# NVlabs/intrinsic3d

Hardware: AMD Instinct MI355X
Metric: Gauss-Newton iterations/s at the finest SDF level (higher is better)
Workload: dtype f32

## Files before the change

### include/intrinsic3d_hip.h

```cpp
#ifndef INTRINSIC3D_HIP_H
#define INTRINSIC3D_HIP_H
#include <stdint.h>
#ifdef __cplusplus
extern "C" {
#endif

typedef struct i3d_context i3d_context;

typedef enum {
    I3D_OK = 0,
    I3D_ERR_INVALID_ARGUMENT = 1,
    I3D_ERR_NO_DEVICE = 2,
    I3D_ERR_HIP = 3,
    I3D_ERR_STATE = 4,
    I3D_ERR_CAPACITY = 5,
    I3D_ERR_COMM = 6,
    I3D_ERR_IO = 7
} i3d_status;

int  i3d_create(int32_t device_ordinal, i3d_context** out);
void i3d_destroy(i3d_context* ctx);
const char* i3d_last_error(const i3d_context* ctx);
const char* i3d_version(void);

// ... 332 lines not shown

typedef struct {
    i3d_track_sdf_stats base;
    int64_t photo_samples;
    double  photo_rms_initial, photo_rms_final;
} i3d_track_sdf_rgbd_stats;

void i3d_track_sdf_rgbd_desc_default(i3d_track_sdf_rgbd_desc* d);
int  i3d_track_frame_sdf_rgbd(i3d_context* ctx, const i3d_track_sdf_rgbd_desc* desc, int32_t width, int32_t height, const float* depth, const float* luminance,
                              double* pose6_io, i3d_track_sdf_rgbd_stats* stats);
int  i3d_fusion_track_sdf_rgbd(i3d_fusion* f, const i3d_track_sdf_rgbd_desc* desc, int32_t width, int32_t height, const float* depth, const float* luminance,
                               double* pose6_io, i3d_track_sdf_rgbd_stats* stats);
int  i3d_track_frames_sdf_rgbd(i3d_context* ctx, const i3d_track_sdf_rgbd_desc* desc, int32_t num_frames, int32_t width, int32_t height,
                               const float* depth, const float* luminance, double* poses6_io, i3d_track_sdf_rgbd_stats* stats);
int  i3d_track_keyframes_sdf_rgbd(i3d_context* ctx, const i3d_track_sdf_rgbd_desc* desc, int32_t level, int32_t num, const int32_t* frames,
                                  double* poses6_io, i3d_track_sdf_rgbd_stats* stats);

int i3d_comm_unique_id(void* out128, int32_t* bytes);
int i3d_comm_init(i3d_context* ctx, int32_t rank, int32_t world, const void* unique_id, int32_t id_bytes);
void* i3d_comm_sim_create(int32_t world);
void  i3d_comm_sim_destroy(void* shared);
int   i3d_comm_init_sim(i3d_context* ctx, void* shared, int32_t rank);
int   i3d_shard_plan(int32_t A, int32_t world, int32_t rank, const int32_t* anbr, const uint8_t* active,
                     int32_t* chunk, int32_t* own0, int32_t* own1, uint8_t* in_compute_list );
int32_t i3d_shard_vec_index(int32_t a, int32_t chunk, int32_t albedo);
int   i3d_shard_need(int32_t A, int32_t world, const int32_t* anbr , const uint8_t* active , uint64_t* need );
int   i3d_comm_stats(i3d_context* ctx, int64_t* halo_calls, int64_t* halo_bytes_sent, int64_t* reduce_calls, int64_t* reduce_bytes,
                     int32_t* halo_entries_send, int32_t* halo_entries_recv, int32_t* ghost_tiles, int32_t* compute_list);
const char* i3d_comm_transport(i3d_context* ctx);

enum { I3D_K_CLASSIFY = 0, I3D_K_OBSERVE, I3D_K_BUILD, I3D_K_EG_PASS , I3D_K_GATHER, I3D_K_COST, I3D_K_VECTOR, I3D_K_SH,
       I3D_K_EG_AUX ,
       I3D_K_COMM ,
       I3D_K_EG_MR2, I3D_K_EG_MR3 , I3D_K_COUNT };
int i3d_timing_enable(i3d_context* ctx, int32_t on);
int i3d_timing_select(i3d_context* ctx, uint32_t category_mask);
int i3d_timing_get(i3d_context* ctx, double* ms , int64_t* launches , int32_t reset);
int i3d_timing_get_work(i3d_context* ctx, double* ms , int64_t* launches );
int i3d_timing_get_work_ex(i3d_context* ctx, double* ms, int64_t* launches, double* slow_ms , int64_t* slow_launches );
const char* i3d_kernel_name(int32_t k);
int i3d_problem_sizes(i3d_context* ctx, int64_t out[6]);

int i3d_debug_assemble(i3d_context* ctx, const i3d_optimizer_config* cfg, int32_t iteration, int32_t* slots_out);
int64_t i3d_debug_map_order(const int32_t* keys, int64_t n, int32_t mode, int32_t* order);
int i3d_debug_flags(i3d_context* ctx, uint8_t* flags );
int i3d_debug_eg_rows(i3d_context* ctx, int32_t* frame , float* weight ,
                      float* residual , float* jac );
int i3d_debug_reg_rows(i3d_context* ctx, uint8_t* has_er , uint8_t* has_es , float* ea_weight );
int i3d_debug_neighbors(i3d_context* ctx, int32_t* nbr );
int i3d_debug_normal_eq(i3d_context* ctx, double* gradient, double* jtj_diag, double* cost);
int i3d_debug_jtj_apply(i3d_context* ctx, const double* x, double* y);
int i3d_debug_work_list(i3d_context* ctx, int32_t* visit_index , int64_t capacity, int64_t* count);
int i3d_debug_counters(i3d_context* ctx, int64_t* stream_syncs);
int i3d_debug_ladder_stats(i3d_context* ctx, int64_t* out6);
int i3d_debug_ladder_passes(i3d_context* ctx, int64_t* out8);
#define I3D_LM_SCRIPT_GUARD 64
typedef struct i3d_lm_script_desc {
    double cost, ngrad, nfree, radius0;
    int32_t lm_steps;
    int32_t K, fix_poses, fix_intr, fix_dist;
    int32_t n_attempts;
    int32_t n_plan, max_setups;
    const double* cdiag;
    const double* tri;
    const float* tail_c; const float* tail_S;
    const double* xbr; const double* d2xx; const int32_t* pcg_it; const int32_t* pcg_done;
    const double* norms2;
    const double* cand_cost; const int32_t* debug_invalid;
    const int32_t* plan;
} i3d_lm_script_desc;
typedef struct i3d_lm_record { int32_t seq, final_, accepted, pcg_it, termination, kind; double cost, cand_cost, model_change, rel, radius_after, ngrad, nfree; } i3d_lm_record;
int i3d_debug_lm_script(i3d_context* ctx, const i3d_lm_script_desc* script, i3d_lm_record* records , int32_t* n_records, double* state25, int32_t* n_setups,
                        int32_t* setup_meta, double* setup_radius, float* setup_inv_radius, float* setup_blocks, float* setup_d2, float* setup_minv);
int i3d_debug_cull_stats(i3d_context* ctx, int64_t* pairs, int64_t* culled);

int i3d_debug_register_sums(i3d_context* ctx, const i3d_register_desc* desc, int64_t n, const double* points, const double* pose6, const double* pivot3,
                            double* sums29, int64_t* valid);
int i3d_debug_register_row_cap(i3d_context* ctx, int32_t rows);
int i3d_debug_track_sdf_sums(i3d_context* ctx, const i3d_track_sdf_desc* desc, int32_t width, int32_t height, const float* depth,
                             const double* pose6 , const double* pivot3, double* sums29, int64_t* valid, int64_t* valid_pixels);
int i3d_debug_track_batch_frames(i3d_context* ctx, int32_t frames_per_chunk);
int i3d_debug_track_sdf_rgbd_sums(i3d_context* ctx, const i3d_track_sdf_rgbd_desc* desc, int32_t width, int32_t height, const float* depth, const float* luminance,
                                  const double* pose6 , const double* pivot3, double* sums31, int64_t* valid, int64_t* photo_samples);
int i3d_debug_voxel_intensity(i3d_context* ctx, int32_t use_refined_sdf, double* c);
int i3d_fusion_debug_voxel_luminance(i3d_fusion* f, int64_t n, const int32_t* keys , double* c );
int i3d_fusion_debug_track_sdf_rgbd_sums(i3d_fusion* f, const i3d_track_sdf_rgbd_desc* desc, int32_t width, int32_t height, const float* depth,
                                         const float* luminance, const double* pose6 , const double* pivot3, double* sums31, int64_t* valid,
                                         int64_t* photo_samples);
int i3d_fusion_debug_voxels(i3d_fusion* f, int64_t n, const int32_t* keys , uint8_t* found, float* sdf, float* weight, uint8_t* color ,
                            int64_t* first_frame);
int i3d_fusion_debug_frame_samples(i3d_fusion* f, int32_t depth_w, int32_t depth_h, const float* depth_intr4, int32_t color_w, int32_t color_h, const float* color_intr4,
                                   const float* depth, const uint8_t* bgr, const float* pose_cam_to_world16, int32_t erode_window, int64_t n,
                                   const int32_t* keys , uint8_t* on, float* sample, float* wu, uint8_t* has_color, uint8_t* rgb );
int i3d_fusion_debug_register_volume_selection(i3d_fusion* src, const i3d_register_volume_desc* desc, int64_t capacity, int32_t* keys ,
                                               float* sdf , int64_t* count);
int i3d_fusion_debug_register_volume_sums(i3d_fusion* f, i3d_fusion* src, const i3d_register_volume_desc* desc, const double* pose6, const double* pivot3,
                                          int64_t limit, int32_t row_cap, double* sums29, int64_t* valid, int64_t* selected);

#ifdef __cplusplus
}
#endif
#endif
```

### intrinsic3d_amd/binding.py

```python
from __future__ import annotations

import ctypes as C
import os

import numpy as np

_HERE = os.path.dirname(os.path.abspath(__file__))
LIB_PATH = os.environ.get("I3D_LIB") or os.path.join(_HERE, "libintrinsic3d_hip.so")

K_NAMES = ["classify", "observe", "build", "eg_pass", "gather", "cost", "vector", "sh", "eg_aux", "comm", "eg_mr2", "eg_mr3"]


class OptimizerConfig(C.Structure):
    _fields_ = [("iterations", C.c_int32), ("lm_steps", C.c_int32),
                ("lambda_g", C.c_double), ("lambda_r0", C.c_double), ("lambda_r1", C.c_double),
                ("lambda_s0", C.c_double), ("lambda_s1", C.c_double), ("lambda_a", C.c_double),
                ("fix_poses", C.c_int32), ("fix_intrinsics", C.c_int32), ("fix_distortion", C.c_int32),
                ("occlusion_distance", C.c_float), ("num_observations", C.c_int32),
                ("thres_shell", C.c_double), ("grid_level", C.c_int32), ("rgbd_level", C.c_int32),
                ("pcg_fixed_iterations", C.c_int32), ("verbose", C.c_int32), ("carry_trust_radius", C.c_int32), ("fix_sdf", C.c_int32)]


class IterationStats(C.Structure):
    _fields_ = [("rows", C.c_int64 * 4), ("weight_sum", C.c_double * 4), ("type_weight", C.c_double * 4),
# ... 878 lines not shown
        self._check(self.L.i3d_timing_get_work_ex(self.h, _p(ms), _p(n), _p(sms), _p(sn)), "i3d_timing_get_work_ex")
        return {k: (ms[i], int(n[i]), sms[i], int(sn[i])) for i, k in enumerate(K_NAMES)}

    def timing_get(self, reset=True):
        ms = np.zeros(len(K_NAMES)); n = np.zeros(len(K_NAMES), np.int64)
        self._check(self.L.i3d_timing_get(self.h, _p(ms), _p(n), 1 if reset else 0), "i3d_timing_get")
        return {k: (ms[i], int(n[i])) for i, k in enumerate(K_NAMES)}

    def problem_sizes(self):
        o = np.zeros(6, np.int64)
        self._check(self.L.i3d_problem_sizes(self.h, _p(o)), "i3d_problem_sizes")
        return dict(zip(["active", "eg", "er", "es", "ea", "free"], [int(x) for x in o]))

    def debug_assemble(self, cfg, iteration=0):
        s = C.c_int32(0)
        self._check(self.L.i3d_debug_assemble(self.h, C.byref(cfg), int(iteration), C.byref(s)), "i3d_debug_assemble")
        self.slots = s.value
        return s.value

    def debug_flags(self):
        f = np.zeros(self.N, np.uint8)
        self._check(self.L.i3d_debug_flags(self.h, _p(f)), "i3d_debug_flags")
        return f

    def debug_eg_rows(self, jac=True):
        S = self.slots
        fr = np.zeros((self.N, S), np.int32); w = np.zeros((self.N, S), np.float32); r = np.zeros((self.N, S), np.float32)
        J = np.zeros((self.N, S, 29), np.float32) if jac else None
        self._check(self.L.i3d_debug_eg_rows(self.h, _p(fr), _p(w), _p(r), _p(J)), "i3d_debug_eg_rows")
        return fr, w, r, J

    def debug_reg_rows(self):
        er = np.zeros(self.N, np.uint8); es = np.zeros(self.N, np.uint8); ea = np.zeros((self.N, 6), np.float32)
        self._check(self.L.i3d_debug_reg_rows(self.h, _p(er), _p(es), _p(ea)), "i3d_debug_reg_rows")
        return er, es, ea

    def debug_neighbors(self):
        nb = np.zeros((self.N, 18), np.int32)
        self._check(self.L.i3d_debug_neighbors(self.h, _p(nb)), "i3d_debug_neighbors")
        return nb

    def debug_normal_eq(self):
        NP = 2 * self.N + 6 * self.K + 9
        g = np.zeros(NP); d = np.zeros(NP); cost = C.c_double(0)
        self._check(self.L.i3d_debug_normal_eq(self.h, _p(g), _p(d), C.byref(cost)), "i3d_debug_normal_eq")
        return g, d, cost.value

    def debug_counters(self):
        n = C.c_int64(0)
        self._check(self.L.i3d_debug_counters(self.h, C.byref(n)), "i3d_debug_counters")
        return {"stream_syncs": int(n.value)}

    def debug_ladder_stats(self):
        a = (C.c_int64 * 6)()
        self._check(self.L.i3d_debug_ladder_stats(self.h, a), "i3d_debug_ladder_stats")
        return {"batches": int(a[0]), "row_streams": int(a[1]), "system_passes": int(a[2]), "resyncs": int(a[3]), "unused_systems": int(a[4]), "depth": int(a[5])}

    def debug_ladder_passes(self):
        a = (C.c_int64 * 8)()
        self._check(self.L.i3d_debug_ladder_passes(self.h, a), "i3d_debug_ladder_passes")
        return {"live": [int(a[n]) for n in range(7)], "paired": int(a[7])}

    def debug_cull_stats(self):
        a = C.c_int64(0); b = C.c_int64(0)
        self._check(self.L.i3d_debug_cull_stats(self.h, C.byref(a), C.byref(b)), "i3d_debug_cull_stats")
        return int(a.value), int(b.value)

    def debug_jtj_apply(self, x):
        x = np.ascontiguousarray(x, np.float64); y = np.zeros_like(x)
        self._check(self.L.i3d_debug_jtj_apply(self.h, _p(x), _p(y)), "i3d_debug_jtj_apply")
        return y

    def debug_lm_script(self, cost, ngrad, nfree, radius0, lm_steps, attempts, plan=(), K=0, fix=(0, 0, 0), cdiag=None, tri=None, tail_c=None, tail_S=None):
        NS, NB, NT, G = 6 * K + 9, 36 * K + 41, 21 * K + 25, LM_SCRIPT_GUARD
        f64 = lambda a, n, fill: np.full(n, fill, np.float64) if a is None else np.ascontiguousarray(a, np.float64).reshape(n)
        f32 = lambda a, n, fill: np.full(n, fill, np.float32) if a is None else np.ascontiguousarray(a, np.float32).reshape(n)
        cdiag = f64(cdiag, NS, 1.0); tail_c = f32(tail_c, NS, 1.0); tail_S = f32(tail_S, NS, 0.5)
        if tri is None:
            tri = np.zeros(NT); o = 0
            for n in [6] * K + [4, 5]:
                d = 0
                for i in range(n):
                    tri[o + d] = 1.0; d += n - i
                o += n * (n + 1) // 2
        tri = f64(tri, NT, 0.0)
        n = len(attempts["xbr"])
        a = {k: np.ascontiguousarray(attempts[k], np.float64) for k in ("xbr", "d2xx", "norms2", "cand_cost")}
        a.update({k: np.ascontiguousarray(attempts[k], np.int32) for k in ("pcg_it", "pcg_done", "debug_invalid")})
        assert all(a[k].size == (2 * n if k == "norms2" else n) for k in a)
        plan = np.ascontiguousarray(plan, np.int32)
        S = 6 * int(lm_steps) + 6 if plan.size else int(lm_steps)
        d = LmScriptDesc(float(cost), float(ngrad), float(nfree), float(radius0), int(lm_steps), int(K), int(fix[0]), int(fix[1]), int(fix[2]), n, int(plan.size), S,
                         cdiag.ctypes.data, tri.ctypes.data, tail_c.ctypes.data, tail_S.ctypes.data, a["xbr"].ctypes.data, a["d2xx"].ctypes.data, a["pcg_it"].ctypes.data,
                         a["pcg_done"].ctypes.data, a["norms2"].ctypes.data, a["cand_cost"].ctypes.data, a["debug_invalid"].ctypes.data, plan.ctypes.data if plan.size else None)
        rec = np.zeros(128, LM_RECORD_DTYPE); nrec = C.c_int32(0); nset = C.c_int32(0); state = np.zeros(25)
        meta = np.zeros((S, 4), np.int32); radius = np.zeros(S); inv_radius = np.zeros(S, np.float32)
        blocks = np.zeros((S, NB + 2 * G), np.float32); d2 = np.zeros((S, NS + 2 * G), np.float32); minv = np.zeros((S, NS + 2 * G), np.float32)
        self._check(self.L.i3d_debug_lm_script(self.h, C.byref(d), _p(rec), C.addressof(nrec), _p(state), C.addressof(nset), _p(meta), _p(radius), _p(inv_radius),
                                               _p(blocks), _p(d2), _p(minv)), "i3d_debug_lm_script")
        ns = int(nset.value)
        names = ["cost", "radius", "decrease_factor", "ngrad", "nfree", "inv_radius", "done", "termination", "accepted", "invalid", "attempts", "successful", "lad_n"]
        st = {k: state[i] for i, k in enumerate(names)}; st["lad_radius"] = state[13:19].copy(); st["lad_inv_radius"] = state[19:25].copy()
        return {"records": rec[:int(nrec.value)].copy(), "state": st, "meta": meta[:ns], "radius": radius[:ns], "inv_radius": inv_radius[:ns],
                "blocks": blocks[:ns], "d2": d2[:ns], "minv": minv[:ns]}

    def debug_work_list(self):
        n = C.c_int64(0)
        self._check(self.L.i3d_debug_work_list(self.h, None, 0, C.byref(n)), "i3d_debug_work_list")
        out = np.zeros(max(int(n.value), 1), np.int32)
# ... 446 lines not shown
```

### intrinsic3d_amd/csrc/device/build.hip

```cpp
#include <type_traits>
#include "kernels.hpp"
#include "reduce_device.hpp"

namespace i3d {

typedef float v4f_row __attribute__((ext_vector_type(4)));
typedef float v2f_row __attribute__((ext_vector_type(2)));
typedef float f2 __attribute__((ext_vector_type(2)));
static __device__ inline void st_row2(float2* p, float a, float b) { v2f_row v; v.x = a; v.y = b; __builtin_nontemporal_store(v, reinterpret_cast<v2f_row*>(p)); }
static __device__ inline void st_row(float4* p, float a, float b, float c, float d) { v4f_row v; v.x = a; v.y = b; v.z = c; v.w = d; __builtin_nontemporal_store(v, reinterpret_cast<v4f_row*>(p)); }

typedef float f4u __attribute__((ext_vector_type(4), aligned(4)));
typedef const __attribute__((address_space(1))) f4u* gf4u_ptr;
typedef const __attribute__((address_space(1))) float* gf_ptr;

constexpr int Q_LDS_STRIDE = 296;
struct PointShared {
    double P[3];
    double B;
    float n[3];
    float inv_len;
    float s;
    float Ls;
    float dLs[3];
// ... 91 lines not shown
    fold_weights<double>(k.map, wc);
    double fr[4];
#pragma unroll
    for (int i = 0; i < 4; ++i) fr[i] = wc[0] * (double)t[i].x + wc[1] * (double)t[i].y + wc[2] * (double)t[i].z + wc[3] * (double)t[i].w;
    f = wr[0] * fr[0] + wr[1] * fr[1] + wr[2] * fr[2] + wr[3] * fr[3];
    if (WITH_J) {
        float dwc[4], dwr[4]; cr_dweights<float>((float)k.xc, dwc); cr_dweights<float>((float)k.xr, dwr);
        fold_weights<float>(k.map, dwc);
        dfdr = dwr[0] * (float)(fr[0] - fr[1]) + dwr[2] * (float)(fr[2] - fr[1]) + dwr[3] * (float)(fr[3] - fr[1]);
        float acc = 0.0f;
#pragma unroll
        for (int i = 0; i < 4; ++i) acc += (float)wr[i] * (dwc[0] * (t[i].x - t[i].y) + dwc[2] * (t[i].z - t[i].y) + dwc[3] * (t[i].w - t[i].y));
        dfdc = acc;
    }
}

struct PointVal {
    float x0, y0, iz, dfdr, dfdc;
};

template <bool WITH_J>
static __device__ inline bool project_point(const double P[3], const double R[9], const double t[3], const OptParams& p, double& u, double& v, PointVal& o) {
    const double X = R[0] * P[0] + R[1] * P[1] + R[2] * P[2] + t[0];
    const double Y = R[3] * P[0] + R[4] * P[1] + R[5] * P[2] + t[1];
    const double Z = R[6] * P[0] + R[7] * P[1] + R[8] * P[2] + t[2];
    const double ps = p.pyr_scale;
    const double iz = rcp64(Z);
    const double x0 = X * iz, y0 = Y * iz;
    const double r2 = x0 * x0 + y0 * y0, r4 = r2 * r2, r6 = r4 * r2;
    const double dc = 1.0 + p.dist[0] * r2 + p.dist[1] * r4 + p.dist[2] * r6;
    const double xd = x0 * dc + 2.0 * p.dist[3] * x0 * y0 + p.dist[4] * (r2 + 2.0 * x0 * x0);
    const double yd = y0 * dc + 2.0 * p.dist[4] * xd * y0 + p.dist[3] * (r2 + 2.0 * y0 * y0);
    u = (p.intr[0] * ps) * xd + p.intr[2] * ps; v = (p.intr[1] * ps) * yd + p.intr[3] * ps;
    if (WITH_J) { o.x0 = (float)x0; o.y0 = (float)y0; o.iz = (float)iz; }
    return u >= 0.0 && u <= (double)(p.w - 1) && v >= 0.0 && v <= (double)(p.h - 1);
}

static __device__ inline double sdf_to_weight(double sdf, double trunc) {
    const double a = fmin(fabs(sdf), trunc) / trunc;
    return fmin(fmax(1.0 - a, 0.01), 1.0);
}
static __device__ inline float chroma_weight(uchar4 c, uchar4 cn) {
    const float s = 1.0f / 255.0f;
    const float lum = 0.299f * (float)c.x + 0.587f * (float)c.y + 0.114f * (float)c.z;
    const float lumn = 0.299f * (float)cn.x + 0.587f * (float)cn.y + 0.114f * (float)cn.z;
    const float a0 = ((float)c.x * s) / lum - ((float)cn.x * s) / lumn;
    const float a1 = ((float)c.y * s) / lum - ((float)cn.y * s) / lumn;
    const float a2 = ((float)c.z * s) / lum - ((float)cn.z * s) / lumn;
    const float d = sqrtf(a0 * a0 + (a1 * a1 + a2 * a2))      ;
    const float one_minus = 1.0f - d;
    return (one_minus < 0.01f) ? 0.01f : one_minus;
}

template <bool WITH_J, bool FR_LDS, int BATCH> __global__ void k_build(GridView g, RowView r, OptParams p, const FrameConst* __restrict__ frames, double* cost_out, const double* __restrict__ cam9, const LmState* __restrict__ lm);
#ifdef I3D_BUILD_VALUE_PROBE
constexpr int BUILD_PROBE_WAVES = I3D_BUILD_VALUE_PROBE;
#else
constexpr int BUILD_PROBE_WAVES = 0;
#endif
template <bool WITH_J, bool FR_LDS, int BATCH>
__global__ void __launch_bounds__(256, WITH_J ? (BUILD_PROBE_WAVES ? BUILD_PROBE_WAVES : 2) : 3) k_build(GridView g, RowView r, OptParams p, const FrameConst* __restrict__ frames, double* cost_out,
                                                               const double* __restrict__ cam9, const LmState* __restrict__ lm) {
    extern __shared__ double frame_lds_raw[];
    if (!WITH_J) {
        if (lm && lm->done) return;
        if (cam9) { for (int i = 0; i < 4; ++i) p.intr[i] = cam9[i]; for (int i = 0; i < 5; ++i) p.dist[i] = cam9[4 + i]; }
    }
    FrameHot* const flds = reinterpret_cast<FrameHot*>(frame_lds_raw);
    if (FR_LDS) {
        constexpr int WORDS = sizeof(FrameHot) / 8;
        for (int i = threadIdx.x; i < p.K * WORDS; i += blockDim.x) {
            const int f = i / WORDS, w = i - f * WORDS;
            frame_lds_raw[(size_t)f * WORDS + w] = reinterpret_cast<const double*>(&frames[f].hot)[w];
        }
        __syncthreads();
    }
#ifdef I3D_COST_MULTI_PROBE
    int bx = blockIdx.x; bool probe_extra = false;
#ifdef I3D_COST_MULTI_PROBE_FAR
    if (!WITH_J) { constexpr int PB = I3D_COST_MULTI_PROBE; const int per = (int)gridDim.x / PB; probe_extra = (int)blockIdx.x / per != 0; bx = (int)blockIdx.x % per; }
#else
    if (!WITH_J) { constexpr int PB = I3D_COST_MULTI_PROBE; const int grp = (int)blockIdx.x / (8 * PB), rr = (int)blockIdx.x % (8 * PB); probe_extra = rr / 8 != 0; bx = grp * 8 + (rr % 8); }
#endif
    const int ci = bx * blockDim.x + threadIdx.x;
#else
    const int ci = blockIdx.x * blockDim.x + threadIdx.x;
#endif
    const int a = ci < r.nC ? (r.clist ? r.clist[ci] : ci) : -1;
    const bool owned = a >= r.own0 && a < r.own1;
    double cost = 0.0;
    if (a >= 0 && (WITH_J || owned)) {
        const int N = g.N; const size_t Acap = r.Acap;
        const int s = r.alist[a];
        const uint8_t fl = r.aflags[a];
        uint8_t pre_rf = 0, pre_eafree = 0, pre_nrows = 0; float eaw[6] = {0.0f, 0.0f, 0.0f, 0.0f, 0.0f, 0.0f};
        if (!WITH_J) {
            pre_rf = r.regflags[a]; pre_eafree = r.ea_free[a]; pre_nrows = r.nrows[a];
#pragma unroll
            for (int d = 0; d < 6; ++d) eaw[d] = r.ea_w[(size_t)d * Acap + a];
        }
        __builtin_amdgcn_sched_barrier(0);
        if (!(fl & F_ACTIVE)) {
            if (WITH_J) {
                r.regflags[a] = 0; r.ea_free[a] = 0; r.nrows[a] = 0;
                for (int d = 0; d < 6; ++d) r.ea_w[(size_t)d * Acap + a] = 0.0f;
            }
        } else {
        int idx[P_VOX];
        bool eligible = true;
#pragma unroll
        for (int c = 0; c < 10; ++c) { const int nb = slot_fwd_nbr(c); idx[c] = nb < 0 ? s : g.nbr[(size_t)nb * N + s]; eligible &= idx[c] >= 0; }
        idx[10] = idx[0]; idx[11] = idx[6]; idx[12] = idx[1]; idx[13] = idx[4];

        int ring[6];
#pragma unroll
        for (int d = 0; d < 6; ++d) ring[d] = g.nbr[(size_t)d * N + s];
        const bool ring_ok = (fl & F_RING) != 0;
        const double xs = g.x_sdf[s];
        uint8_t rf = 0;
        if (WITH_J) {
            uint8_t nfl[6]; int nrk[6]; uchar4 ncol[6];
#pragma unroll
            for (int d = 0; d < 6; ++d) { const int nb = ring_ok ? ring[d] : s; nfl[d] = g.flags[nb]; nrk[d] = g.rank[nb]; ncol[d] = g.color[nb]; }
            const uchar4 col = g.color[s];
            const int myrank = g.rank[s];
            const double sdf0s = g.sdf0[s];
            if (p.use_er && ring_ok) {
                rf |= 1;
                bool fr = (fl & F_FREE_SDF) != 0;
#pragma unroll
                for (int d = 0; d < 6; ++d) fr |= (nfl[d] & F_FREE_SDF) != 0;
                if (fr) rf |= 8;
            }
            if (p.use_es) { rf |= 2; if ((xs - sdf0s) != 0.0) rf |= 4; if (fl & F_FREE_SDF) rf |= 16; }
            uint8_t eafree = 0;
#pragma unroll
            for (int d = 0; d < 6; ++d) {
                float w = 0.0f;
                if (p.use_ea && ring_ok) {
                    const bool added_before = (nfl[d] & F_ACTIVE) && nrk[d] < myrank;
// ... 191 lines not shown
                    const f2 dyd_dy0 = dc + 2.0f * y0 * y0 * dcr + 2.0f * k4 * (xd + y0 * dxd_dy0) + 6.0f * k3 * y0;
                    const f2 au = dfdc * fxs, av = dfdr * fys;
                    const f2 lx = au * dxd_dx0 + av * dyd_dx0, ly = au * dxd_dy0 + av * dyd_dy0;
                    const f2 L0 = lx * iz, L1 = ly * iz, L2 = -(lx * x0 + ly * y0) * iz;
                    const f2 M0 = L0 * R0 + L1 * R3 + L2 * R6, M1 = L0 * R1 + L1 * R4 + L2 * R7, M2 = L0 * R2 + L1 * R5 + L2 * R8;
                    const f2 c = {cj[ja], cj[jb]};
                    const f2 alb = {q[ja].alb, q[jb].alb}, sv = {q[ja].s, q[jb].s}, il = {q[ja].inv_len, q[jb].inv_len};
                    const f2 n0 = {q[ja].n[0], q[jb].n[0]}, n1 = {q[ja].n[1], q[jb].n[1]}, n2 = {q[ja].n[2], q[jb].n[2]};
                    const f2 v0 = alb * f2{q[ja].dLs[0], q[jb].dLs[0]} + sv * M0, v1 = alb * f2{q[ja].dLs[1], q[jb].dLs[1]} + sv * M1, v2 = alb * f2{q[ja].dLs[2], q[jb].dLs[2]} + sv * M2;
                    const f2 d = n0 * v0 + n1 * v1 + n2 * v2;
                    f2 G0 = (v0 - n0 * d) * il, G1 = (v1 - n1 * d) * il, G2 = (v2 - n2 * d) * il;
                    if (il.x == 0.0f) { G0.x = v0.x; G1.x = v1.x; G2.x = v2.x; }
                    if (il.y == 0.0f) { G0.y = v0.y; G1.y = v1.y; G2.y = v2.y; }
                    const f2 direct = M0 * n0 + M1 * n1 + M2 * n2;
                    const f2 cG0 = c * G0, cG1 = c * G1, cG2 = c * G2, cD = c * (direct - (G0 + G1 + G2)), cLs = c * f2{q[ja].Ls, q[jb].Ls};
                    J[PS[ja][1]] += cG0.x; J[PS[ja][2]] += cG1.x; J[PS[ja][3]] += cG2.x; J[PS[ja][0]] += cD.x; J[P_ALB + ja] = cLs.x;
                    J[PS[jb][1]] += cG0.y; J[PS[jb][2]] += cG1.y; J[PS[jb][3]] += cG2.y; J[PS[jb][0]] += cD.y; J[P_ALB + jb] = cLs.y;
                    const f2 cL0 = c * L0, cL1 = c * L1, cL2 = c * L2;
                    J[P_POSE + 3] -= cL0.x + cL0.y; J[P_POSE + 4] -= cL1.x + cL1.y; J[P_POSE + 5] -= cL2.x + cL2.y;
                    const f2 Px = {(float)q[ja].P[0], (float)q[jb].P[0]}, Py = {(float)q[ja].P[1], (float)q[jb].P[1]}, Pz = {(float)q[ja].P[2], (float)q[jb].P[2]};
                    const f2 wx = c * (Py * M2 - Pz * M1), wy = c * (Pz * M0 - Px * M2), wz = c * (Px * M1 - Py * M0);
                    Wx += wx.x + wx.y; Wy += wy.x + wy.y; Wz += wz.x + wz.y;
                    const f2 cdc = c * dfdc * psf, cdr = c * dfdr * psf;
                    const f2 i0 = cdc * xd, i1 = cdr * yd;
                    J[P_INTR + 0] -= i0.x + i0.y; J[P_INTR + 1] -= i1.x + i1.y; J[P_INTR + 2] -= cdc.x + cdc.y; J[P_INTR + 3] -= cdr.x + cdr.y;
                    const f2 dxk0 = x0 * r2, dxk1 = x0 * r4, dxk2 = x0 * r6, dxk3 = 2.0f * x0 * y0, dxk4 = r2 + 2.0f * x0 * x0;
                    const f2 c2 = 2.0f * k4 * y0;
                    const f2 e0 = c * (au * dxk0 + av * (y0 * r2 + c2 * dxk0)), e1 = c * (au * dxk1 + av * (y0 * r4 + c2 * dxk1)), e2 = c * (au * dxk2 + av * (y0 * r6 + c2 * dxk2));
                    const f2 e3 = c * (au * dxk3 + av * (c2 * dxk3 + (r2 + 2.0f * y0 * y0))), e4 = c * (au * dxk4 + av * (2.0f * xd * y0 + c2 * dxk4));
                    J[P_DIST + 0] -= e0.x + e0.y; J[P_DIST + 1] -= e1.x + e1.y; J[P_DIST + 2] -= e2.x + e2.y; J[P_DIST + 3] -= e3.x + e3.y; J[P_DIST + 4] -= e4.x + e4.y;
                }
                J[P_POSE + 0] = -(Wx * jr[0] + Wy * jr[3] + Wz * jr[6]);
                J[P_POSE + 1] = -(Wx * jr[1] + Wy * jr[4] + Wz * jr[7]);
                J[P_POSE + 2] = -(Wx * jr[2] + Wy * jr[5] + Wz * jr[8]);
                float finz = 0.0f;
#pragma unroll
                for (int i = 0; i < P_TOTAL; ++i) finz = __builtin_fmaf(J[i], 0.0f, finz);
                if (!(finz == 0.0f)) continue;
#pragma unroll
                for (int gq = 0; gq < 7; ++gq)
                    st_row(&r.rows[row_index(a, nout, gq, r.slots)], J[4 * gq], J[4 * gq + 1], J[4 * gq + 2], J[4 * gq + 3]);
                const size_t ro = row_scalar_index(a, nout, r.slots);
                st_row2(&r.row_jt()[row_jt_index(a, nout, r.slots)], J[28], __int_as_float(f | (vox_free ? ROW_FREE_BIT : 0)));
                st_row2(&r.row_wr[ro], roww, (float)res);
                ++nout;
            }
            }
        }
        if (WITH_J) {
            r.nrows[a] = (uint8_t)nout;
        }
        }
    }
#ifdef I3D_COST_MULTI_PROBE
    if (!WITH_J && probe_extra) cost = 0.0;
#endif
    if (!WITH_J) block_partial_d(cost, cost_out, 1, 0);
}

void launch_build(hipStream_t st, GridView g, RowView r, OptParams p, const FrameConst* frames, bool with_jacobian, double* cost_out, double* scratch,
                  const double* cam9, const LmState* lm) {
    if (r.nC <= 0) { if (!with_jacobian && cost_out) (void)hipMemsetAsync(cost_out, 0, sizeof(double), st); return; }
#ifdef I3D_COST_MULTI_PROBE
    const int blocks = with_jacobian ? (r.nC + 255) / 256 : (((r.nC + 255) / 256 + 7) / 8) * 8 * I3D_COST_MULTI_PROBE;
#else
    const int blocks = (r.nC + 255) / 256;
#endif
    double* const cost_dst = cost_out; cost_out = scratch;
    const size_t lds = (size_t)p.K * sizeof(FrameHot), qlds = (size_t)256 * Q_LDS_STRIDE;
    if (with_jacobian) {
#ifdef I3D_BUILD_VALUE_PROBE
        if (BUILD_PROBE_WAVES > 2) {
            if (!set_dynamic_lds((const void*)k_build<true, true, 2>, "k_build<true> value probe", lds, p.K)) return;
            k_build<true, true, 2><<<blocks, 256, lds, st>>>(g, r, p, frames, cost_out, nullptr, nullptr);
            return;
        }
#endif
        if (!set_dynamic_lds((const void*)k_build<true, false, 2>, "k_build<true>", qlds, p.K)) return;
        k_build<true, false, 2><<<blocks, 256, qlds, st>>>(g, r, p, frames, cost_out, nullptr, nullptr);
    } else {
        if (lds <= 48 * 1024) k_build<false, true, 2><<<blocks, 256, lds, st>>>(g, r, p, frames, cost_out, cam9, lm);
        else k_build<false, false, 2><<<blocks, 256, 0, st>>>(g, r, p, frames, cost_out, cam9, lm);
    }
    if (!with_jacobian) launch_reduce_partials(st, scratch, blocks, 1, cost_dst, nullptr, true);
}

template <bool COST>
__global__ void __launch_bounds__(256) k_weight_sums(RowView r, GridView g, double* partials) {
    double s0 = 0, s1 = 0, s2 = 0, s3 = 0, n0 = 0, n3 = 0, na = 0, c0 = 0, c1 = 0, c2 = 0, c3 = 0;
    const int N = g.N;
    for (int a = r.own0 + blockIdx.x * blockDim.x + threadIdx.x; a < r.own1 && a < r.A; a += gridDim.x * blockDim.x) {
        if (!(r.aflags[a] & F_ACTIVE)) continue;
        na += 1.0;
        const int nr = r.nrows[a];
        for (int k = 0; k < nr; ++k) {
            const float2 wr = r.row_wr[row_scalar_index(a, k, r.slots)]; const float w = wr.x;
            s0 += (double)w; if (w != 0.0f) n0 += 1.0;
            if (COST && (__float_as_int(r.row_jt()[row_jt_index(a, k, r.slots)].y) & ROW_FREE_BIT)) c0 += (double)w * ((double)wr.y * (double)wr.y);
        }
        const uint8_t rf = r.regflags[a];
        if (rf & 1) s1 += 1.0;
        if (rf & 2) s2 += 1.0;
        const int s = COST ? r.alist[a] : 0;
        const uint8_t eafree = COST ? r.ea_free[a] : 0;
        const bool er = COST && (rf & 1) && (rf & 8), es = COST && (rf & 2) && (rf & 16);
        int ring[6];
        if (er || eafree) {
#pragma unroll
            for (int d = 0; d < 6; ++d) ring[d] = g.nbr[(size_t)d * N + s];
        }
        if (er || es) {
            const double xs = g.x_sdf[s];
            if (er) {
                const double dxx = g.x_sdf[ring[0]] + g.x_sdf[ring[1]] - 2.0 * xs, dyy = g.x_sdf[ring[2]] + g.x_sdf[ring[3]] - 2.0 * xs, dzz = g.x_sdf[ring[4]] + g.x_sdf[ring[5]] - 2.0 * xs;
                const double lap = dxx + dyy + dzz; c1 += lap * lap;
            }
            if (es) { double e = xs - g.sdf0[s]; if (e == 0.0) e = 0.0000001; c2 += e * e; }
        }
        const double xa = eafree ? g.x_alb[s] : 0.0;
#pragma unroll
        for (int d = 0; d < 6; ++d) {
            const float w = r.ea_w[(size_t)d * r.Acap + a]; s3 += (double)w; if (w != 0.0f) n3 += 1.0;
            if (eafree & (1 << d)) { const double e = xa - g.x_alb[ring[d]]; c3 += (double)w * (e * e); }
        }
    }
    block_partial_d(s0, partials, 13, 0); block_partial_d(s1, partials, 13, 1); block_partial_d(s2, partials, 13, 2); block_partial_d(s3, partials, 13, 3);
    block_partial_d(n0, partials, 13, 4); block_partial_d(0.0, partials, 13, 5); block_partial_d(0.0, partials, 13, 6); block_partial_d(n3, partials, 13, 7);
    block_partial_d(na, partials, 13, 8);
    block_partial_d(c0, partials, 13, 9); block_partial_d(c1, partials, 13, 10); block_partial_d(c2, partials, 13, 11); block_partial_d(c3, partials, 13, 12);
}
void launch_weight_sums(hipStream_t st, RowView r, GridView g, bool with_cost, double* sums13, double* scratch) {
    const int n = r.own1 - r.own0;
    if (n <= 0) return;
    int blocks = (n + 255) / 256; if (blocks > 1024) blocks = 1024;
    if (with_cost) k_weight_sums<true><<<blocks, 256, 0, st>>>(r, g, scratch);
    else k_weight_sums<false><<<blocks, 256, 0, st>>>(r, g, scratch);
    launch_reduce_partials(st, scratch, blocks, 13, sums13, nullptr);
// ... 4 lines not shown
```

### intrinsic3d_amd/csrc/device/common.hpp

```cpp
#pragma once
#include <hip/hip_runtime.h>
#include <cstdint>
#include <cstdio>

namespace i3d {

constexpr int NUM_NBR = 18;
enum Nbr { NB_PX = 0, NB_MX, NB_PY, NB_MY, NB_PZ, NB_MZ, NB_P2X, NB_P2Y, NB_P2Z, NB_PXY, NB_PXZ, NB_PYZ,
           NB_M2X, NB_M2Y, NB_M2Z, NB_MXY, NB_MXZ, NB_MYZ };
__host__ __device__ inline void nbr_offset(int i, int& dx, int& dy, int& dz) {
    constexpr int8_t O[NUM_NBR][3] = {{1,0,0},{-1,0,0},{0,1,0},{0,-1,0},{0,0,1},{0,0,-1},{2,0,0},{0,2,0},{0,0,2},{1,1,0},{1,0,1},{0,1,1},
                                      {-2,0,0},{0,-2,0},{0,0,-2},{-1,-1,0},{-1,0,-1},{0,-1,-1}};
    dx = O[i][0]; dy = O[i][1]; dz = O[i][2];
}

constexpr int P_SDF = 0, P_ALB = 10, P_POSE = 14, P_INTR = 20, P_DIST = 24, P_TOTAL = 29, P_VOX = 14;
__host__ __device__ inline int slot_fwd_nbr(int c) {
    constexpr int8_t F[P_VOX] = {-1, NB_PY, NB_P2Y, NB_PYZ, NB_PZ, NB_P2Z, NB_PX, NB_PXY, NB_PXZ, NB_P2X, -1, NB_PX, NB_PY, NB_PZ};
    return F[c];
}
__host__ __device__ inline int slot_rev_nbr(int c) {
    constexpr int8_t R[P_VOX] = {-1, NB_MY, NB_M2Y, NB_MYZ, NB_MZ, NB_M2Z, NB_MX, NB_MXY, NB_MXZ, NB_M2X, -1, NB_MX, NB_MY, NB_MZ};
    return R[c];
}
// ... 62 lines not shown
}

struct RowView {
    int A; int Acap; int slots;
    int chunk;
    int world;
    int own0, own1;
    const int* clist; int nC;
    const int* alist;
    const uint8_t* aflags;
    const int* anbr;
    int* obs_frame; float* obs_w;
    float4* rows; float2* row_wr;
    __host__ __device__ float2* row_jt() const { return reinterpret_cast<float2*>(rows); }
    uint8_t* nrows;
    int* gmax;
    uint8_t* regflags;
    float* ea_w;
    uint8_t* ea_free;
};

#ifdef __HIPCC__
static __device__ inline float lm_scale(float cm) { return cm >= 0.0f ? __builtin_amdgcn_rcpf(1.0f + __builtin_amdgcn_sqrtf(cm)) : 0.0f; }
static __device__ inline void lm_diag(float cm, float s, float inv_radius, float& d2, float& minv) {
    if (s == 0.0f) { d2 = 0.0f; minv = 0.0f; return; }
    const float cs = (cm * s) * s;
    d2 = fminf(fmaxf(cs, 1e-6f), 1e32f) * inv_radius; minv = __builtin_amdgcn_rcpf(cs + d2);
}
#endif

struct PcgState {
    double acc[4];
    double rho, last_rho, pq, alpha, beta;
    double xbr, xr, d2xx;
    double Q0, Q1;
    int it;
    int done;
    int fixed_iterations;
    int max_iterations;
};

constexpr int LADDER_MAX = 6;
struct LmState {
    double cost;
    double radius, decrease_factor;
    double ngrad, nfree;
    float  inv_radius; int pad0;
    int done;
    int termination;
    int accepted;
    int invalid;
    int attempts;
    int successful;
    double lad_radius[LADDER_MAX]; float lad_inv_radius[LADDER_MAX]; int lad_n; int pad1;
};
struct LmRecord {
    int seq; int final_;
    int accepted; int pcg_it; int termination; int kind;
    double cost, cand_cost, model_change, rel, radius_after, ngrad, nfree;
};

struct OptParams {
    double thres_shell; double lambda_a;
    double type_w[4];
    float type_wf[4];
    int K; int level; double pyr_scale; float occlusion; int use_er, use_es, use_ea;
    double intr[4]; double dist[5];
    float cam_f[4]; float dist_f[5]; int dist_zero; int w, h;
    int fix_poses, fix_intr, fix_dist, fix_sdf;
};

#define I3D_HIP_CHECK(expr) do { hipError_t _e = (expr); if (_e != hipSuccess) { \
    std::snprintf(i3d::g_errbuf, sizeof(i3d::g_errbuf), "%s:%d %s -> %s", __FILE__, __LINE__, #expr, hipGetErrorString(_e)); return I3D_ERR_HIP_; } } while (0)
constexpr int I3D_ERR_HIP_ = 3;
extern thread_local char g_errbuf[512];

constexpr size_t I3D_LDS_LIMIT = 160 * 1024;
bool set_dynamic_lds(const void* kernel, const char* name, size_t bytes, int K);
bool take_launch_error(char* msg, size_t n);

}
```

### intrinsic3d_amd/csrc/device/kernels.hpp

```cpp
#pragma once
#include "common.hpp"
#include "p2p_device.hpp"

namespace i3d {

struct HashTable { unsigned long long* keys; int* vals; unsigned int mask; };
void launch_sort_keys(hipStream_t st, int N, const int* keys_xyz , unsigned long long* sort_keys, int* iota);
void launch_permute_grid(hipStream_t st, int N, const int* perm, const int* keys_xyz, const double* sdf, const double* sdf_ref,
                         const double* alb, const float* w, const uint8_t* rgb,
                         int* cx, int* cy, int* cz, int* rank, double* sdf0, double* x_sdf, double* x_alb, float* f_sdf, float* f_alb,
                         float* weight, uchar4* color);
void launch_hash_build(hipStream_t st, int N, const int* cx, const int* cy, const int* cz, HashTable t);
void launch_nbr_build(hipStream_t st, int N, const int* cx, const int* cy, const int* cz, HashTable t, int* nbr);
void launch_classify(hipStream_t st, GridView g, OptParams p, int* active_flag);
void launch_compact(hipStream_t st, int N, const int* active_flag, const int* active_scan, const uint8_t* flags, int* aidx, int* alist, uint8_t* aflags);
void launch_partition_blocks(hipStream_t st, GridView g, int A, int* alist, uint8_t* aflags, int* aidx);
void launch_group_rows(hipStream_t st, int A, const uint8_t* nrows, int* gmax);
void launch_anbr(hipStream_t st, int N, int A, int Acap, const int* alist, const int* nbr, const int* aidx, int* anbr);
void launch_scatter_sh(hipStream_t st, int N, const int* rank, const double* sh_visit , float* sh );
void launch_gather_visit(hipStream_t st, int N, const int* rank, const double* x_sdf, const double* x_alb, double* out_sdf, double* out_alb);
void launch_update_fields(hipStream_t st, int N, const int* rank, const double* sdf_ref, const double* alb, const uint8_t* rgb,
                          double* x_sdf, double* x_alb, float* f_sdf, float* f_alb, uchar4* color);

void launch_observe(hipStream_t st, GridView g, RowView r, OptParams p, const FrameConst* frames, const unsigned* cull_mask = nullptr, bool prefilter = false);
constexpr int CULL_BLOCK = 8, CULL_MAX_LEVELS = 12;
struct CullPyramid { int levels, cells; int bw[CULL_MAX_LEVELS], bh[CULL_MAX_LEVELS], off[CULL_MAX_LEVELS]; };
CullPyramid cull_pyramid(int w, int h);
void launch_depth_blocks(hipStream_t st, const FrameConst* frames, int K, int w, int h, float2* out);
void launch_group_cull(hipStream_t st, GridView g, RowView r, OptParams p, const FrameConst* frames, const float2* dblocks, float4* bounds, unsigned* mask);

void launch_build(hipStream_t st, GridView g, RowView r, OptParams p, const FrameConst* frames, bool with_jacobian, double* cost_out , double* scratch,
                  const double* cam9 = nullptr, const LmState* lm = nullptr);
void launch_weight_sums(hipStream_t st, RowView r, GridView g, bool with_cost, double* sums13 , double* scratch);

enum PassMode { PASS_GRAD = 0, PASS_JTJP = 1, PASS_COLNORM = 2 };
struct Seg2 { size_t off0, off1; int n; };
struct PassBuffers {
    float* C;
    float* treg;
    double* shared;
    double* blocks;
    float* part; int part_stride;
};
struct GradColBuffers {
    float* Cg; float* Cc;
    float* tregg; float* tregc;
    float* part; int part_stride;
    int col_off;
    double* cost_partials; double* cost_out;
};
int  launch_eg_gradcol(hipStream_t st, GridView g, RowView r, OptParams p, GradColBuffers b);
int  launch_eg_pass(hipStream_t st, PassMode mode, GridView g, RowView r, OptParams p, const float* u , PassBuffers b, const PcgState* state);
void launch_sum_rows(hipStream_t st, PassMode mode, int K, const float* part, int nrows, int stride, double* shared, double* blocks);
void launch_gather(hipStream_t st, PassMode mode, RowView r, PassBuffers b, float* out );
int  launch_gather_tail(hipStream_t st, RowView r, PassBuffers b, float* out, const float* S, const float* D2, const float* v, double* dot_partials ,
                        bool dot_atomic, const PcgState* state);
void launch_reduce_partials(hipStream_t st, const double* partials, int nblk, int ncomp, double* dst, const PcgState* state, bool assign = false);
void launch_shared_finalize(hipStream_t st, size_t tail_off, int K, OptParams p, const double* shared, float* out , bool tail, const float* S, const float* D2,
                            const float* v, double* dot_out, const PcgState* state);

void launch_fill(hipStream_t st, int n, float* x, float v);
void launch_fill_d(hipStream_t st, int n, double* x, double v);
void launch_int_to_double(hipStream_t st, const int* src, double* dst);
void launch_mul(hipStream_t st, int n, const float* a, const float* b, float* out);
void launch_scale_from_colnorm(hipStream_t st, int n, const float* c, const float* freemask, float* S, float* cm);
void launch_dot(hipStream_t st, int n, const float* a, const float* b, double* out , double* scratch);
void launch_count_above2(hipStream_t st, Seg2 sg, const float* a, const float* m, float tol, double* out, double* scratch);
void launch_count_above(hipStream_t st, int n, const float* a, const float* m, float tol, double* out, double* scratch);
void launch_dot2(hipStream_t st, Seg2 sg, const float* a, const float* b, double* out , double* scratch);
void launch_mul2(hipStream_t st, Seg2 sg, const float* a, const float* b, float* out);
void launch_freemask(hipStream_t st, RowView r, OptParams p, float* mask );

void launch_pcg_init(hipStream_t st, PcgState* state, int fixed_iterations, int max_iterations, const LmState* lm = nullptr);
int  launch_pcg_step(hipStream_t st, int mode, Seg2 sg, const float* p, const float* q, float* x, float* r, const float* b, const float* D2, const float* Minv,
                     float* z, const float* S_for_inline_q, double* partials , PcgState* state);
void launch_pcg_tail_x(hipStream_t st, size_t tail_off, int K, const float* p, float* x, const PcgState* state);
void launch_pcg_tail_a(hipStream_t st, int mode, size_t tail_off, int K, const float* Minv_blocks, const float* p, const float* q, float* x, float* r, const float* b,
                       const float* D2, float* z, const double* partials, int nblk, PcgState* state,
                       double* shared_zero, int nzero, int* host_flags, int seq,
                       const P2PDev& pd);
int  launch_pcg_direction(hipStream_t st, Seg2 sg, size_t tail_off, int ntail, const float* z, float* p, const float* S, float* u, const float* D2,
                          double* d2_partials , const PcgState* state);
void launch_pcg_tail_b(hipStream_t st, size_t tail_off, int K, OptParams p, double* shared, const double* pq_slice, const double* pq_partials, int nblk,
                       const double* pq_partials2, int nblk2, bool rowwise,
                       float* q, const float* S, const float* D2, const float* v, PcgState* state, const P2PDev& pd);
// ... 39 lines not shown
};
struct LadVec {
    size_t vec;
    size_t qh;
    size_t cam;
    size_t part;
    size_t mblk;
    size_t tail;
    int sysid[LADDER_MAX];
};
struct Step3Args {
    int nq; int chunk4;
    const float4* p; const float4* qacc; float4* x; float4* r; const float4* b; float4* z;
    const float4* cm; const LmState* lm;
    const int* ext_off; const int* ext_pos; const float2* qh; int e0;
    const double* pq_partials; int n_pq; const double* d2_partials; int n_d2;
    int n_slice_wg;
    int K; int fix_poses, fix_intr, fix_dist;
    const float* cam_partials; int n_cam; int cam_stride; const float* Mblk;
    const float* tp; float* tx; float* tr; const float* tb; const float* tD2; float* tz; const float* tS;
    double* step_partials;
    PcgState* cur;
    int sharded; ShardArgs sh;
    int lad_sys;
    const double* redop; int redop_stride;
};
void launch_pcg_init3(hipStream_t st, PcgState* st2 , int fixed_iterations, int max_iterations, const LmState* lm = nullptr);
int  launch_pcg_dir3(hipStream_t st, bool init, Seg2 sg, size_t tail_off, int ntail, const float* z, float* p, const float* S, float* u, const float* D2, const float* cm, const LmState* lm,
                     const double* step_partials, int n_step, double* d2_partials, const PcgState* prev, PcgState* next, int* host_flags, int seq,
                     const ShardArgs* sa = nullptr);
void launch_rim_u(hipStream_t st, const ShardArgs& sa, const PcgState* state);
int  pcg_step3_slice_wgs(int n_entries, int cap = 0);
int  pcg_step3_tail_wgs(int K);
int  launch_pcg_step3(hipStream_t st, int mode , Step3Args a);
void launch_halo_fold(hipStream_t st, RowView r, TilePlan t, float* qacc, const PcgState* state);
void launch_pcg_init_lad(hipStream_t st, PcgState* st2_all , int B, int fixed_iterations, int max_iterations, const LmState* lm);
int  launch_pcg_dir3_lad(hipStream_t st, bool init, int nsys, Seg2 sg, size_t tail_off, int ntail, const float* z0, float* p0, const float* S, float* u0, const float* tD2_0, const float* cm, const LmState* lm,
                         const double* step_partials0, int n_step, double* d2_partials0, PcgState* st2_0, int prev_parity, int* host_flags0, int seq, const LadVec& lv,
                         int n_slice_partials = 0, const double* red4_0 = nullptr );
int  launch_pcg_step3_lad(hipStream_t st, int mode, int nsys, Step3Args a, const LadVec& lv);
void launch_lad_reduce_step(hipStream_t st, int nsys, const double* step_partials0, int n_slice, double* red4_0, const LadVec& lv);
void launch_lad_reduce_op(hipStream_t st, int nsys, const float* cam_partials0, int n_cam, int cam_stride, int NS, const double* pq_partials0, int n_pq, const double* d2_partials0, int n_d2,
                          double* redop0, int redop_stride, const LadVec& lv);

void launch_need_mask(hipStream_t st, RowView r, int slice, unsigned long long* need );
void launch_halo_items(hipStream_t st, int A, int slice, int me, const unsigned long long* need, unsigned long long* items, int* count , int cap);
void launch_tile_flags(hipStream_t st, int A, int T, const int* cflag, int* tileflag );
size_t halo_sort_temp_bytes(int cap);
hipError_t launch_halo_sort(hipStream_t st, void* temp, size_t temp_bytes, const unsigned long long* in, unsigned long long* out, int n);

void launch_candidate(hipStream_t st, GridView g, RowView r, int K, float sign, const float* step, const float* S, const double* x_shared, double* xc_sdf, double* xc_alb,
                      double* xc_shared, double* norms2 , const float* mask, double* scratch, const LmState* lm = nullptr);
void launch_accept(hipStream_t st, GridView g, RowView r, const double* xc_sdf, const double* xc_alb, const LmState* lm = nullptr);
void launch_set_double(hipStream_t st, double* dst, double v);
void launch_lm_init(hipStream_t st, LmState* lm, const double* cost, const double* ngrad, const double* nfree, double radius0, LmRecord* rec, int seq);
void launch_lm_begin(hipStream_t st, LmState* lm, int K, int fix_poses, int fix_intr, int fix_dist, const double* cdiag, const double* tri, float* Mblk,
                     const float* tc, const float* tS, float* tD2, float* tMinv, LmRecord* rec, int seq);
void launch_lm_diag_dev(hipStream_t st, int n, const float* c, const float* S, const LmState* lm, float* D2, float* Minv);
void launch_cand_frames(hipStream_t st, int K, const double* xc, const FrameConst* base, FrameConst* out, const LmState* lm);
void launch_lm_decide(hipStream_t st, LmState* lm, const PcgState* ps, const double* norms2, const double* cand_cost, int attempt, int lm_steps, LmRecord* rec, int seq,
                      int lad_next = -1 , int debug_invalid = 0);
void launch_lm_begin_lad(hipStream_t st, LmState* lm, int B, int K, int fix_poses, int fix_intr, int fix_dist, const double* cdiag, const double* tri, float* Mblk, size_t mblk_stride,
                         const float* tc, const float* tS, float* tD2, size_t tail_stride, LmRecord* rec, int seq);
void launch_mark_compute(hipStream_t st, RowView r, int* flag);
void launch_compact_list(hipStream_t st, int A, const int* flag, const int* scan, int* list);

}
```

### intrinsic3d_amd/csrc/device/lm_kernels.hip

```cpp
#include "kernels.hpp"
#include "frame_math.hpp"

namespace i3d {

static __device__ inline void lm_publish(LmRecord* rec, int seq) {
    if (rec) __hip_atomic_store(&rec->seq, seq, __ATOMIC_RELEASE, __HIP_MEMORY_SCOPE_SYSTEM);
}

__global__ void k_lm_init(LmState* lm, const double* __restrict__ cost, const double* __restrict__ ngrad, const double* __restrict__ nfree, double radius0, LmRecord* rec, int seq) {
    LmState s;
    s.cost = *cost; s.radius = radius0; s.decrease_factor = 2.0; s.ngrad = *ngrad; s.nfree = *nfree;
    s.inv_radius = (float)(1.0 / radius0); s.pad0 = 0;
    s.done = 0; s.termination = 0; s.accepted = 0; s.invalid = 0; s.attempts = 0; s.successful = 0;
    if (s.nfree == 0.0 || s.ngrad == 0.0) { s.done = 1; s.termination = 1; }
    *lm = s;
    if (rec) {
        rec->final_ = s.done; rec->accepted = 0; rec->pcg_it = 0; rec->termination = s.termination; rec->kind = 0;
        rec->cost = s.cost; rec->cand_cost = 0.0; rec->model_change = 0.0; rec->rel = 0.0; rec->radius_after = s.radius; rec->ngrad = s.ngrad; rec->nfree = s.nfree;
        lm_publish(rec, seq);
    }
}
__global__ void k_set_double(double* dst, double v) { *dst = v; }
void launch_set_double(hipStream_t st, double* dst, double v) { k_set_double<<<1, 1, 0, st>>>(dst, v); }
void launch_lm_init(hipStream_t st, LmState* lm, const double* cost, const double* ngrad, const double* nfree, double radius0, LmRecord* rec, int seq) {
// ... 59 lines not shown
    if (lm->done == 1) return;
    const int j = blockIdx.y, gid = blockIdx.x * blockDim.x + threadIdx.x;
    double radius = lm->radius, dec = lm->decrease_factor;
    if (j == 0 && radius < 1e-32) {
        if (gid == 0) {
            lm->termination = 1; lm->done = 1; lm->lad_n = 0;
            if (rec) { rec->final_ = 1; rec->accepted = 0; rec->pcg_it = 0; rec->termination = 1; rec->kind = 2; rec->cost = lm->cost; rec->cand_cost = 0.0; rec->model_change = 0.0; rec->rel = 0.0;
                       rec->radius_after = radius; rec->ngrad = lm->ngrad; rec->nfree = lm->nfree; lm_publish(rec, seq); }
        }
        return;
    }
    for (int s = 0; s < j; ++s) { radius = radius / dec; dec *= 2.0; }
    const bool dead = radius < 1e-32;
    const float inv_radius = dead ? 0.0f : (float)(1.0 / radius);
    if (gid == 0) { lm->lad_radius[j] = radius; lm->lad_inv_radius[j] = inv_radius; if (j == 0) { lm->lad_n = B; lm->inv_radius = inv_radius; lm->done = 0; } }
    if (dead) return;
    float* const Mb = Mblk + (size_t)j * mblk_stride;
    if (gid < K) cam_block_inverse(6, cdiag + 6 * gid, tri + 21 * gid, fix_poses != 0, radius, Mb + 36 * (size_t)gid);
    else if (gid == K) cam_block_inverse(4, cdiag + 6 * K, tri + 21 * K, fix_intr != 0, radius, Mb + 36 * (size_t)K);
    else if (gid == K + 1) cam_block_inverse(5, cdiag + 6 * K + 4, tri + 21 * K + 10, fix_dist != 0, radius, Mb + 36 * (size_t)K + 16);
    const int NS = 6 * K + 9;
    for (int i = gid; i < NS; i += gridDim.x * blockDim.x) { float d2, mi; lm_diag(tc[i], tS[i], inv_radius, d2, mi); tD2[(size_t)j * tail_stride + i] = d2; }
}
void launch_lm_begin_lad(hipStream_t st, LmState* lm, int B, int K, int fix_poses, int fix_intr, int fix_dist, const double* cdiag, const double* tri, float* Mblk, size_t mblk_stride,
                         const float* tc, const float* tS, float* tD2, size_t tail_stride, LmRecord* rec, int seq) {
    k_lm_begin_lad<<<dim3((K + 2 + 63) / 64, B), 64, 0, st>>>(lm, B, K, fix_poses, fix_intr, fix_dist, cdiag, tri, Mblk, mblk_stride, tc, tS, tD2, tail_stride, rec, seq);
}

__global__ void k_lm_diag_dev(int n, const float* __restrict__ c, const float* __restrict__ S, const LmState* __restrict__ lm, float* __restrict__ D2, float* __restrict__ Minv) {
    if (lm->done) return;
    const float ir = lm->inv_radius;
    for (int i = blockIdx.x * blockDim.x + threadIdx.x; i < n; i += gridDim.x * blockDim.x) { float d2, mi; lm_diag(c[i], S[i], ir, d2, mi); D2[i] = d2; Minv[i] = mi; }
}
void launch_lm_diag_dev(hipStream_t st, int n, const float* c, const float* S, const LmState* lm, float* D2, float* Minv) {
    if (n <= 0) return;
    int b = (n + 255) / 256; b = b > 2048 ? 2048 : b;
    k_lm_diag_dev<<<b, 256, 0, st>>>(n, c, S, lm, D2, Minv);
}

__global__ void __launch_bounds__(64) k_cand_frames(int K, const double* __restrict__ xc, const FrameConst* __restrict__ base, FrameConst* __restrict__ out, const LmState* __restrict__ lm) {
    if (lm->done) return;
    const int f = blockIdx.x * blockDim.x + threadIdx.x;
    if (f >= K) return;
    FrameConst fc = base[f];
    double p[6];
    for (int i = 0; i < 6; ++i) p[i] = xc[6 * f + i];
    fm::frame_from_pose(p, fc);
    out[f] = fc;
}
void launch_cand_frames(hipStream_t st, int K, const double* xc, const FrameConst* base, FrameConst* out, const LmState* lm) {
    if (K > 0) k_cand_frames<<<(K + 63) / 64, 64, 0, st>>>(K, xc, base, out, lm);
}

__global__ void k_lm_decide(LmState* lm, const PcgState* __restrict__ ps, const double* __restrict__ norms2, const double* __restrict__ cand_cost_p, int attempt , int lm_steps,
                            LmRecord* rec, int seq, int lad_next, int debug_invalid) {
    if (lm->done) return;
    const int pcg_it = ps->done == 2 ? ps->it + 1 : ps->it;
    const double xbr = ps->xbr, d2xx = ps->d2xx;
    const double model_change = 0.5 * xbr + 0.5 * d2xx;
    const bool finite = !(isnan(xbr) || isinf(xbr) || isnan(d2xx) || isinf(d2xx));
    double radius = lm->radius, decrease = lm->decrease_factor, cost = lm->cost;
    const double cand = *cand_cost_p;
    int final_ = 0, accepted = 0, termination = lm->termination, invalid = lm->invalid, successful = lm->successful;
    double rel = 0.0;
    if (!finite || !(model_change > 0.0) || debug_invalid) {
        if (++invalid >= 5) { termination = 3; final_ = 1; }
        else radius *= 0.5;
    } else {
        invalid = 0;
        const double step_norm = sqrt(norms2[0]), x_norm = sqrt(norms2[1]);
        const double cost_change = cost - cand;
        if (step_norm <= 1e-8 * (x_norm + 1e-8)) { termination = 1; final_ = 1; }
        else if (fabs(cost_change) <= 1e-6 * cost) { termination = 1; final_ = 1; }
        else {
            rel = cost_change / model_change;
            if (rel > 1e-3) {
                accepted = 1; cost = cand;
                radius = fmin(1e16, radius / fmax(1.0 / 3.0, 1.0 - pow(2.0 * rel - 1.0, 3.0)));
                decrease = 2.0;
                successful += 1; termination = 2; final_ = 1;
            } else { radius = radius / decrease; decrease *= 2.0; }
        }
    }
    if (!final_ && attempt + 1 >= lm_steps) final_ = 1;
    lm->radius = radius; lm->decrease_factor = decrease; lm->cost = cost; lm->invalid = invalid; lm->successful = successful; lm->termination = termination;
    lm->attempts = lm->attempts + 1; lm->accepted = accepted; lm->done = final_;
    if (rec) {
        rec->final_ = final_; rec->accepted = accepted; rec->pcg_it = pcg_it; rec->termination = termination; rec->kind = 1;
        rec->cost = cost; rec->cand_cost = cand; rec->model_change = model_change; rec->rel = rel; rec->radius_after = radius; rec->ngrad = lm->ngrad; rec->nfree = lm->nfree;
        lm_publish(rec, seq);
    }
    if (!final_ && lad_next >= 0 && lad_next < lm->lad_n) {
        LmRecord* const nrec = rec ? rec + 1 : nullptr;
        if (radius != lm->lad_radius[lad_next]) {
            lm->done = 2;
            if (nrec) { nrec->final_ = 0; nrec->accepted = 0; nrec->pcg_it = 0; nrec->termination = termination; nrec->kind = 3; nrec->cost = cost; nrec->cand_cost = 0.0; nrec->model_change = 0.0;
                        nrec->rel = 0.0; nrec->radius_after = radius; nrec->ngrad = lm->ngrad; nrec->nfree = lm->nfree; lm_publish(nrec, seq + 1); }
        } else if (radius < 1e-32) {
            lm->termination = 1; lm->done = 1;
            if (nrec) { nrec->final_ = 1; nrec->accepted = 0; nrec->pcg_it = 0; nrec->termination = 1; nrec->kind = 2; nrec->cost = cost; nrec->cand_cost = 0.0; nrec->model_change = 0.0;
                        nrec->rel = 0.0; nrec->radius_after = radius; nrec->ngrad = lm->ngrad; nrec->nfree = lm->nfree; lm_publish(nrec, seq + 1); }
        }
    }
}
void launch_lm_decide(hipStream_t st, LmState* lm, const PcgState* ps, const double* norms2, const double* cand_cost, int attempt, int lm_steps, LmRecord* rec, int seq, int lad_next, int debug_invalid) {
    k_lm_decide<<<1, 1, 0, st>>>(lm, ps, norms2, cand_cost, attempt, lm_steps, rec, seq, lad_next, debug_invalid);
}

}
```

### intrinsic3d_amd/csrc/device/operator.hip

```cpp
#include "kernels.hpp"
#include "reduce_device.hpp"
#include "wave_ops.hpp"

namespace i3d {

#define GRID_STRIDE(n) const int stride = gridDim.x * blockDim.x; for (int i = blockIdx.x * blockDim.x + threadIdx.x; i < (n); i += stride)
static inline int vblocks(int n) { int b = (n + 255) / 256; return b < 1 ? 1 : (b > 2048 ? 2048 : b); }

__global__ void __launch_bounds__(1024) k_reduce_partials(const double* __restrict__ partials, int nblk, int ncomp, double* dst, const PcgState* __restrict__ state, int assign) {
    if (state && state->done) return;
    for (int k = 0; k < ncomp; ++k) {
        double s = 0.0;
        for (int i0 = threadIdx.x; i0 < nblk; i0 += 8 * 1024) {
            double v[8];
#pragma unroll
            for (int q = 0; q < 8; ++q) v[q] = partials[(size_t)min(i0 + q * 1024, nblk - 1) * ncomp + k];
#pragma unroll
            for (int q = 0; q < 8; ++q) if (i0 + q * 1024 < nblk) s += v[q];
        }
        const double t = block_sum_d(s);
        if (threadIdx.x == 0) dst[k] = assign ? t : dst[k] + t;
    }
}
void launch_reduce_partials(hipStream_t st, const double* partials, int nblk, int ncomp, double* dst, const PcgState* state, bool assign) {
    if (nblk > 0) k_reduce_partials<<<1, 1024, 0, st>>>(partials, nblk, ncomp, dst, state, assign ? 1 : 0);
}

constexpr int EG_THREADS = 1024;

template <int MODE>
__global__ void __launch_bounds__(EG_THREADS) k_eg_pass(GridView g, RowView r, OptParams p, PassBuffers b, int tiles_per_block, const PcgState* __restrict__ state) {
    static_assert(MODE == PASS_GRAD || MODE == PASS_COLNORM, "the operator pass has its own kernel");
    if (state && state->done) return;
    extern __shared__ float lds[];
    const int K = p.K; const size_t Acap = r.Acap;
    constexpr int NPVT = (MODE == PASS_COLNORM) ? 21 : 6, TCT = (MODE == PASS_COLNORM) ? 16 : 32, NWT = EG_THREADS / 64;
    const int rs = ((MODE == PASS_COLNORM) ? 21 * K : 6 * K) | 1;
    constexpr int NCAM = (MODE == PASS_COLNORM) ? 34 : 9;
    constexpr int D_CAMW = 4, D_TAG = D_CAMW + ((NWT * NCAM + 3) & ~3), D_VAL = D_TAG + NWT * TCT, D0 = D_VAL + NWT * TCT * NPVT;
    const int nacc = D0 + rs + NCAM;
    for (int i = threadIdx.x; i < nacc; i += EG_THREADS) lds[i] = (i >= D_TAG && i < D_VAL) ? __int_as_float(-1) : 0.0f;
    __syncthreads();
    const int wave = __builtin_amdgcn_readfirstlane((int)(threadIdx.x >> 6));
    const int o_tag = D_TAG + wave * TCT, o_val = D_VAL + wave * (TCT * NPVT);
    int tcount = 0;
    float* const cam_acc = lds + D0 + rs;
    float cam9[9];
#pragma unroll
    for (int i = 0; i < 9; ++i) cam9[i] = 0.0f;
    float camb[NCAM];
#pragma unroll
    for (int i = 0; i < NCAM; ++i) camb[i] = 0.0f;
    const float tw0 = (float)p.type_w[0];
    const int nC = r.nC;
    const int ntiles = (nC + EG_THREADS - 1) / EG_THREADS;
    const int tile0 = blockIdx.x * tiles_per_block;

    for (int tile = tile0; tile < tile0 + tiles_per_block && tile < ntiles; ++tile) {
        const int ci = tile * EG_THREADS + threadIdx.x;
        const bool in = ci < nC;
        const int a = in ? (r.clist ? r.clist[ci] : ci) : 0;
        const bool owned = in && a >= r.own0 && a < r.own1;
        const uint8_t fl = in ? r.aflags[a] : 0;
        const int nr = (in && (fl & F_ACTIVE)) ? (int)r.nrows[a] : 0;
        int nr_max = nr;
        for (int o = 32; o > 0; o >>= 1) nr_max = max(nr_max, __shfl_xor(nr_max, o, 64));

        float acc[P_VOX];
#pragma unroll
        for (int c = 0; c < P_VOX; ++c) acc[c] = 0.0f;
        const size_t ac = in ? (size_t)a : 0;
        for (int k = 0; k < nr_max; ++k) {
            const float4* __restrict__ row = r.rows + row_index(ac, k, 0, r.slots);
            float4 j4[7];
#pragma unroll
// ... 707 lines not shown
                       const float* D2, float* z, const double* partials, int nblk, PcgState* state, double* shared_zero, int nzero, int* host_flags, int seq, const P2PDev& pd) {
    k_pcg_tail_a<<<1, 1024, 0, st>>>(mode, tail_off, K, Minv_blocks, p, q, x, r, b, D2, z, partials, nblk, state, shared_zero, nzero, host_flags, seq, pd);
}
int launch_pcg_direction(hipStream_t st, Seg2 sg, size_t tail_off, int ntail, const float* z, float* p, const float* S, float* u, const float* D2, double* d2_partials,
                         const PcgState* state) {
    if (sg.n <= 0 && ntail <= 0) return 0;
    const int n4 = sg.n >> 2, seg4 = (int)((sg.off1 - sg.off0) >> 2);
    const int blocks = step_blocks(2 * n4 > 0 ? 2 * n4 : 1);
    const size_t o = sg.off0;
    k_pcg_direction<<<blocks, 256, 0, st>>>(n4, seg4, tail_off - o, ntail, z + o, p + o, S + o, u + o, D2 + o, d2_partials, state);
    return d2_partials ? blocks : 0;
}
void launch_pcg_tail_b(hipStream_t st, size_t tail_off, int K, OptParams p, double* shared, const double* pq_slice, const double* pq_partials, int nblk,
                       const double* pq_partials2, int nblk2, bool rowwise, float* q, const float* S, const float* D2, const float* v, PcgState* state, const P2PDev& pd) {
    k_pcg_tail_b<<<1, 1024, 0, st>>>(tail_off, K, p, shared, pq_slice, pq_partials, nblk, pq_partials2, nblk2, rowwise ? 1 : 0, q, S, D2, v, state, pd);
}

__global__ void __launch_bounds__(256) k_candidate(GridView g, RowView r, int K, float sign, const float* __restrict__ step, const float* __restrict__ S,
                                                   const double* __restrict__ xsh, double* xc_sdf, double* xc_alb, double* xc_sh,
                                                   double* norms2, const float* __restrict__ mask, const LmState* __restrict__ lm) {
    if (lm && lm->done) return;
    const int A = r.A, NS = 6 * K + 9, chunk = r.chunk;
    const size_t tail = 2 * (size_t)chunk;
    double d2 = 0.0, x2 = 0.0;
    GRID_STRIDE(A + NS) {
        if (i < A) {
            const int s = r.alist[i]; const int js = vec_sdf(i, chunk), ja = js + chunk;
            const double ds = (double)sign * (double)step[js] * (double)S[js], da = (double)sign * (double)step[ja] * (double)S[ja];
            const double xs = g.x_sdf[s], xa = g.x_alb[s];
            xc_sdf[s] = xs + ds; xc_alb[s] = xa + da;
            if (mask[js] != 0.0f) { d2 += ds * ds; x2 += xs * xs; }
            if (mask[ja] != 0.0f) { d2 += da * da; x2 += xa * xa; }
        } else {
            const int t = i - A; const size_t j = tail + t;
            const double delta = (double)sign * (double)step[j] * (double)S[j];
            const double x = xsh[t]; xc_sh[t] = x + delta;
            if (mask[j] != 0.0f) { d2 += delta * delta; x2 += x * x; }
        }
    }
    block_partial_d(d2, norms2, 2, 0); block_partial_d(x2, norms2, 2, 1);
}
void launch_candidate(hipStream_t st, GridView g, RowView r, int K, float sign, const float* step, const float* S, const double* xsh, double* xc_sdf, double* xc_alb,
                      double* xc_sh, double* norms2, const float* mask, double* scratch, const LmState* lm) {
    int b = vblocks(r.A + 6 * K + 9); if (b > 1024) b = 1024;
    k_candidate<<<b, 256, 0, st>>>(g, r, K, sign, step, S, xsh, xc_sdf, xc_alb, xc_sh, scratch, mask, lm);
    launch_reduce_partials(st, scratch, b, 2, norms2, nullptr, true);
}
__global__ void k_accept(GridView g, RowView r, const double* __restrict__ xc_sdf, const double* __restrict__ xc_alb, const LmState* __restrict__ lm) {
    if (lm && !lm->accepted) return;
    GRID_STRIDE(r.A) { const int s = r.alist[i]; const double a = xc_sdf[s], b = xc_alb[s]; g.x_sdf[s] = a; g.x_alb[s] = b; g.f_sdf[s] = (float)a; g.f_alb[s] = (float)b; }
}
void launch_accept(hipStream_t st, GridView g, RowView r, const double* xc_sdf, const double* xc_alb, const LmState* lm) { if (r.A > 0) k_accept<<<vblocks(r.A), 256, 0, st>>>(g, r, xc_sdf, xc_alb, lm); }

__global__ void k_halo_pack(int n, const int* __restrict__ idx, const float* __restrict__ vec, int chunk, float* __restrict__ buf) {
    const int i = blockIdx.x * blockDim.x + threadIdx.x;
    if (i < n) { const int e = idx[i]; buf[2 * (size_t)i] = vec[e]; buf[2 * (size_t)i + 1] = vec[(size_t)chunk + e]; }
}
__global__ void k_halo_unpack(int n, const int* __restrict__ idx, const float* __restrict__ buf, int chunk, float* __restrict__ vec) {
    const int i = blockIdx.x * blockDim.x + threadIdx.x;
    if (i < n) { const int e = idx[i]; vec[e] = buf[2 * (size_t)i]; vec[(size_t)chunk + e] = buf[2 * (size_t)i + 1]; }
}
__global__ void k_halo_pack_multi(int n, const int* __restrict__ idx, const float* __restrict__ vec0, size_t stride, HaloSys sys, int nsys, int chunk, float* __restrict__ buf) {
    const int i = blockIdx.x * blockDim.x + threadIdx.x;
    if (i >= n * nsys) return;
    const int j = i / nsys, s = i - j * nsys, e = idx[j];
    const float* v = vec0 + (size_t)sys.id[s] * stride;
    buf[2 * (size_t)i] = v[e]; buf[2 * (size_t)i + 1] = v[(size_t)chunk + e];
}
__global__ void k_halo_unpack_multi(int n, const int* __restrict__ idx, const float* __restrict__ buf, size_t stride, HaloSys sys, int nsys, int chunk, float* __restrict__ vec0) {
    const int i = blockIdx.x * blockDim.x + threadIdx.x;
    if (i >= n * nsys) return;
    const int j = i / nsys, s = i - j * nsys, e = idx[j];
    float* v = vec0 + (size_t)sys.id[s] * stride;
    v[e] = buf[2 * (size_t)i]; v[(size_t)chunk + e] = buf[2 * (size_t)i + 1];
}
void launch_halo_pack_multi(hipStream_t st, int n, const int* idx, const float* vec0, size_t stride, HaloSys sys, int nsys, int chunk, float* buf) {
    if (n > 0 && nsys > 0) k_halo_pack_multi<<<(n * nsys + 255) / 256, 256, 0, st>>>(n, idx, vec0, stride, sys, nsys, chunk, buf);
}
void launch_halo_unpack_multi(hipStream_t st, int n, const int* idx, const float* buf, size_t stride, HaloSys sys, int nsys, int chunk, float* vec0) {
    if (n > 0 && nsys > 0) k_halo_unpack_multi<<<(n * nsys + 255) / 256, 256, 0, st>>>(n, idx, buf, stride, sys, nsys, chunk, vec0);
}
void launch_halo_pack(hipStream_t st, int n, const int* idx, const float* vec, int chunk, float* buf) { if (n > 0) k_halo_pack<<<(n + 255) / 256, 256, 0, st>>>(n, idx, vec, chunk, buf); }
void launch_halo_unpack(hipStream_t st, int n, const int* idx, const float* buf, int chunk, float* vec) { if (n > 0) k_halo_unpack<<<(n + 255) / 256, 256, 0, st>>>(n, idx, buf, chunk, vec); }

__global__ void k_mark_compute(RowView r, int* __restrict__ flag) {
    const int a = blockIdx.x * blockDim.x + threadIdx.x;
    if (a >= r.A) return;
    flag[a] = shard_needs_entry(a, r.own0, r.own1, (r.aflags[a] & F_ACTIVE) != 0, r.anbr, r.Acap) ? 1 : 0;
}
void launch_mark_compute(hipStream_t st, RowView r, int* flag) { if (r.A > 0) k_mark_compute<<<(r.A + 255) / 256, 256, 0, st>>>(r, flag); }
__global__ void k_compact_list(int A, const int* __restrict__ flag, const int* __restrict__ scan, int* __restrict__ list) {
    const int a = blockIdx.x * blockDim.x + threadIdx.x;
    if (a < A && flag[a]) list[scan[a]] = a;
}
void launch_compact_list(hipStream_t st, int A, const int* flag, const int* scan, int* list) { if (A > 0) k_compact_list<<<(A + 255) / 256, 256, 0, st>>>(A, flag, scan, list); }

}
```

### intrinsic3d_amd/csrc/host/capi.cpp

```cpp
#include <cstdlib>
#include "context.hpp"

using namespace i3d;

extern "C" {

int i3d_optimize(i3d_context* c, const i3d_optimizer_config* cfg, i3d_iteration_stats* stats) {
    if (!c || !cfg) return ctx_fail(c, I3D_ERR_INVALID_ARGUMENT, "i3d_optimize: null argument");
    return optimize(c, *cfg, stats);
}

int i3d_optimize_host(int32_t device_ordinal, const i3d_optimizer_config* cfg, const i3d_grid_view* grid,
                      double* sdf_refined_io, double* albedo_io, int32_t num_frames, int32_t levels, const int32_t* widths,
                      const int32_t* heights, const float* const* lum, const float* const* depth,
                      double* intr_io, double* dist_io, double* poses_io, const double* voxel_sh, i3d_iteration_stats* stats) {
    if (!cfg || !grid || !sdf_refined_io || !albedo_io || !intr_io || !dist_io || !poses_io || !voxel_sh) return I3D_ERR_INVALID_ARGUMENT;
    i3d_context* c = nullptr;
    int rc = i3d_create(device_ordinal, &c); if (rc) return rc;
    i3d_grid_view gv = *grid; gv.sdf_refined = sdf_refined_io; gv.albedo = albedo_io;
    rc = i3d_set_grid(c, &gv);
    if (!rc) rc = i3d_set_frames(c, num_frames, levels, widths, heights, lum, depth, nullptr);
    if (!rc) rc = i3d_set_camera(c, intr_io, dist_io, poses_io);
    if (!rc) rc = i3d_set_voxel_sh(c, voxel_sh);
    if (!rc) rc = i3d_optimize(c, cfg, stats);
// ... 118 lines not shown
    }
    return I3D_OK;
}

int i3d_debug_reg_rows(i3d_context* c, uint8_t* has_er, uint8_t* has_es, float* ea_weight) {
    if (!c || !c->assembled) return ctx_fail(c, I3D_ERR_STATE, "i3d_debug_reg_rows: not assembled");
    const int N = c->N, A = c->A; const size_t Acap = c->Acap;
    std::vector<int> rank(N), alist(A > 0 ? A : 1); std::vector<uint8_t> rf(Acap), afl(Acap); std::vector<float> ew(Acap * 6);
    CTX_HIP(c, hipMemcpy(rank.data(), c->rank.p, sizeof(int) * (size_t)N, hipMemcpyDeviceToHost));
    if (A > 0) CTX_HIP(c, hipMemcpy(alist.data(), c->alist.p, sizeof(int) * (size_t)A, hipMemcpyDeviceToHost));
    CTX_HIP(c, hipMemcpy(rf.data(), c->regflags.p, Acap, hipMemcpyDeviceToHost));
    CTX_HIP(c, hipMemcpy(afl.data(), c->aflags.p, Acap, hipMemcpyDeviceToHost));
    CTX_HIP(c, hipMemcpy(ew.data(), c->ea_w.p, sizeof(float) * Acap * 6, hipMemcpyDeviceToHost));
    for (int v = 0; v < N; ++v) { if (has_er) has_er[v] = 0; if (has_es) has_es[v] = 0; if (ea_weight) for (int d = 0; d < 6; ++d) ea_weight[(size_t)v * 6 + d] = 0.0f; }
    const float tw = (float)c->last_params.type_w[3];
    for (int a = 0; a < A; ++a) {
        if (!(afl[a] & F_ACTIVE)) continue;
        const int v = rank[alist[a]];
        if (has_er) has_er[v] = rf[a] & 1;
        if (has_es) has_es[v] = (rf[a] >> 1) & 1;
        if (ea_weight) for (int d = 0; d < 6; ++d) ea_weight[(size_t)v * 6 + d] = ew[(size_t)d * Acap + a] * tw;
    }
    return I3D_OK;
}

int i3d_debug_neighbors(i3d_context* c, int32_t* nbr) {
    if (!c || !nbr || !c->have_grid) return ctx_fail(c, I3D_ERR_STATE, "i3d_debug_neighbors: no grid");
    const int N = c->N; std::vector<int> rank(N), t((size_t)NUM_NBR * N);
    CTX_HIP(c, hipMemcpy(rank.data(), c->rank.p, sizeof(int) * (size_t)N, hipMemcpyDeviceToHost));
    CTX_HIP(c, hipMemcpy(t.data(), c->nbr.p, sizeof(int) * (size_t)NUM_NBR * N, hipMemcpyDeviceToHost));
    for (int s = 0; s < N; ++s) for (int i = 0; i < NUM_NBR; ++i) { const int n = t[(size_t)i * N + s]; nbr[(size_t)rank[s] * NUM_NBR + i] = n < 0 ? -1 : rank[n]; }
    return I3D_OK;
}

int i3d_debug_normal_eq(i3d_context* c, double* gradient, double* jtj_diag, double* cost) {
    if (!c) return I3D_ERR_INVALID_ARGUMENT;
    return normal_eq_debug(c, gradient, jtj_diag, cost);
}
int i3d_debug_jtj_apply(i3d_context* c, const double* x, double* y) {
    if (!c || !x || !y) return ctx_fail(c, I3D_ERR_INVALID_ARGUMENT, "i3d_debug_jtj_apply: null pointer");
    return jtj_apply_debug(c, x, y);
}
int i3d_debug_work_list(i3d_context* c, int32_t* visit_index, int64_t capacity, int64_t* count) {
    if (!c) return I3D_ERR_INVALID_ARGUMENT;
    if (!visit_index && !count) return ctx_fail(c, I3D_ERR_INVALID_ARGUMENT, "i3d_debug_work_list: null pointer");
    return work_list_debug(c, visit_index, capacity, count);
}
int i3d_debug_counters(i3d_context* c, int64_t* stream_syncs) {
    if (!c) return I3D_ERR_INVALID_ARGUMENT;
    if (stream_syncs) *stream_syncs = (int64_t)c->n_syncs;
    return I3D_OK;
}

int i3d_debug_ladder_stats(i3d_context* c, int64_t* out6) {
    if (!c || !out6) return I3D_ERR_INVALID_ARGUMENT;
    out6[0] = c->lad_batches; out6[1] = c->lad_streams; out6[2] = c->lad_system_passes; out6[3] = c->lad_resyncs; out6[4] = c->lad_wasted; out6[5] = c->ladder_max;
    return I3D_OK;
}
int i3d_debug_ladder_passes(i3d_context* c, int64_t* out8) {
    if (!c || !out8) return I3D_ERR_INVALID_ARGUMENT;
    for (int n = 0; n < 7; ++n) out8[n] = c->lad_pass_live[n];
    out8[7] = c->lad_paired;
    return I3D_OK;
}

int i3d_debug_cull_stats(i3d_context* c, int64_t* pairs, int64_t* culled) {
    if (!c || !pairs || !culled) return I3D_ERR_INVALID_ARGUMENT;
    if (!c->cull_mask.p || c->nC <= 0) return ctx_fail(c, I3D_ERR_STATE, "i3d_debug_cull_stats: nothing assembled");
    const size_t ngroups = ((size_t)c->nC + 63) / 64, ncw = ((size_t)c->K + 31) / 32;
    *pairs = (int64_t)(ngroups * (size_t)c->K);
    if (!c->cull_on) { *culled = -1; return I3D_OK; }
    std::vector<unsigned> m(ngroups * ncw);
    CTX_HIP(c, hipSetDevice(c->device));
    CTX_HIP(c, hipMemcpy(m.data(), c->cull_mask.p, m.size() * sizeof(unsigned), hipMemcpyDeviceToHost));
    int64_t n = 0; for (unsigned w : m) n += __builtin_popcount(w);
    *culled = n;
    return I3D_OK;
}

}
```

### intrinsic3d_amd/csrc/host/context.cpp

```cpp
#include "context.hpp"
#include "../device/frame_math.hpp"
#include <rocprim/rocprim.hpp>
#include <algorithm>

using namespace i3d;

static thread_local std::string g_create_error;

namespace i3d {

int ctx_fail(i3d_context* c, int code, const std::string& msg) { if (c) c->err = msg; else g_create_error = msg; return code; }
int ctx_hip(i3d_context* c, hipError_t e, const char* what) {
    return ctx_fail(c, I3D_ERR_HIP, std::string(what) + " -> " + hipGetErrorString(e));
}

int ctx_launch_check(i3d_context* c) {
    char msg[256];
    if (take_launch_error(msg, sizeof(msg))) return ctx_fail(c, I3D_ERR_CAPACITY, msg);
    const hipError_t e = hipGetLastError();
    return e == hipSuccess ? I3D_OK : ctx_hip(c, e, "kernel launch");
}

int ensure_pinned(i3d_context* c, size_t n) {
    if (n <= c->h_pinned_n) return I3D_OK;
// ... 89 lines not shown
    if (c->h_pcg) (void)hipHostFree(c->h_pcg);
    if (c->h_flags) (void)hipHostFree(c->h_flags);
    if (c->h_lmrec) (void)hipHostFree(c->h_lmrec);
    for (auto e : c->ev_asm) if (e) (void)hipEventDestroy(e);
    for (auto e : c->pcg_ev) if (e) (void)hipEventDestroy(e);
    delete c->comm;
    if (c->stream) (void)hipStreamDestroy(c->stream);
    delete c;
}

int i3d_set_grid(i3d_context* c, const i3d_grid_view* gv) {
    if (!c || !gv || gv->num_voxels <= 0 || !gv->keys || !gv->sdf || !gv->sdf_refined || !gv->albedo || !gv->weight || !gv->color)
        return ctx_fail(c, I3D_ERR_INVALID_ARGUMENT, "i3d_set_grid: null grid or empty voxel list");
    if (gv->num_voxels > (1ll << 30)) return ctx_fail(c, I3D_ERR_CAPACITY, "i3d_set_grid: more than 2^30 voxels");
    CTX_HIP(c, hipSetDevice(c->device));
    const int N = (int)gv->num_voxels;
    hipStream_t st = c->stream;
    GridStaging g;
    CTX_HIP(c, g.kxyz.alloc((size_t)3 * N)); CTX_HIP(c, g.sdf.alloc(N)); CTX_HIP(c, g.sdf_ref.alloc(N)); CTX_HIP(c, g.alb.alloc(N)); CTX_HIP(c, g.w.alloc(N)); CTX_HIP(c, g.rgb.alloc((size_t)3 * N));
    CTX_HIP(c, hipMemcpyAsync(g.kxyz.p, gv->keys, sizeof(int) * 3 * (size_t)N, hipMemcpyHostToDevice, st));
    CTX_HIP(c, hipMemcpyAsync(g.sdf.p, gv->sdf, sizeof(double) * (size_t)N, hipMemcpyHostToDevice, st));
    CTX_HIP(c, hipMemcpyAsync(g.sdf_ref.p, gv->sdf_refined, sizeof(double) * (size_t)N, hipMemcpyHostToDevice, st));
    CTX_HIP(c, hipMemcpyAsync(g.alb.p, gv->albedo, sizeof(double) * (size_t)N, hipMemcpyHostToDevice, st));
    CTX_HIP(c, hipMemcpyAsync(g.w.p, gv->weight, sizeof(float) * (size_t)N, hipMemcpyHostToDevice, st));
    CTX_HIP(c, hipMemcpyAsync(g.rgb.p, gv->color, (size_t)3 * N, hipMemcpyHostToDevice, st));
    return set_grid_device(c, N, gv->voxel_size, gv->truncation, g);
}

}

namespace i3d {
int set_grid_device(i3d_context* c, int N, float voxel_size, float truncation, GridStaging& g) {
    c->N = N; c->voxel_size = voxel_size; c->truncation = truncation; c->have_grid = false; c->have_sh = false; c->have_subvolumes = false; c->assembled = false;
    c->render_bricks_ok = false;
    c->slots = 0;
    hipStream_t st = c->stream;
    DevBuf<int> perm, iota; DevBuf<unsigned long long> skeys, skeys2;
    CTX_HIP(c, perm.alloc(N)); CTX_HIP(c, iota.alloc(N)); CTX_HIP(c, skeys.alloc(N)); CTX_HIP(c, skeys2.alloc(N));
    launch_sort_keys(st, N, g.kxyz.p, skeys.p, iota.p);
    size_t tmp_bytes = 0;
    CTX_HIP(c, rocprim::radix_sort_pairs(nullptr, tmp_bytes, skeys.p, skeys2.p, iota.p, perm.p, (size_t)N, 0, 64, st));
    DevBuf<unsigned char> tmp; CTX_HIP(c, tmp.alloc(tmp_bytes));
    CTX_HIP(c, rocprim::radix_sort_pairs(tmp.p, tmp_bytes, skeys.p, skeys2.p, iota.p, perm.p, (size_t)N, 0, 64, st));
    auto fit = [&](auto& buf, size_t n) -> hipError_t { if (buf.n != n) buf.release(); return buf.alloc(n); };
    CTX_HIP(c, fit(c->cx, N)); CTX_HIP(c, fit(c->cy, N)); CTX_HIP(c, fit(c->cz, N)); CTX_HIP(c, fit(c->rank, N));
    CTX_HIP(c, fit(c->sdf0, N)); CTX_HIP(c, fit(c->x_sdf, N)); CTX_HIP(c, fit(c->x_alb, N)); CTX_HIP(c, fit(c->xc_sdf, N)); CTX_HIP(c, fit(c->xc_alb, N));
    CTX_HIP(c, fit(c->f_sdf, N)); CTX_HIP(c, fit(c->f_alb, N)); CTX_HIP(c, fit(c->weight, N)); CTX_HIP(c, fit(c->color, N));
    CTX_HIP(c, fit(c->flags, N)); CTX_HIP(c, fit(c->aidx, N)); CTX_HIP(c, fit(c->alist, N)); CTX_HIP(c, fit(c->aflag, N)); CTX_HIP(c, fit(c->ascan, N));
    CTX_HIP(c, fit(c->sh, (size_t)9 * N)); CTX_HIP(c, fit(c->nbr, (size_t)NUM_NBR * N));
    launch_permute_grid(st, N, perm.p, g.kxyz.p, g.sdf.p, g.sdf_ref.p, g.alb.p, g.w.p, g.rgb.p, c->cx.p, c->cy.p, c->cz.p, c->rank.p, c->sdf0.p,
                        c->x_sdf.p, c->x_alb.p, c->f_sdf.p, c->f_alb.p, c->weight.p, c->color.p);
    CTX_HIP(c, hipMemcpyAsync(c->xc_sdf.p, c->x_sdf.p, sizeof(double) * (size_t)N, hipMemcpyDeviceToDevice, st));
    CTX_HIP(c, hipMemcpyAsync(c->xc_alb.p, c->x_alb.p, sizeof(double) * (size_t)N, hipMemcpyDeviceToDevice, st));
    unsigned int cap = 1; while (cap < (unsigned int)N * 2u) cap <<= 1;
    CTX_HIP(c, fit(c->hkeys, cap)); CTX_HIP(c, fit(c->hvals, cap)); c->hmask = cap - 1;
    CTX_HIP(c, hipMemsetAsync(c->hkeys.p, 0xff, sizeof(unsigned long long) * (size_t)cap, st));
    HashTable t{c->hkeys.p, c->hvals.p, cap - 1};
    launch_hash_build(st, N, c->cx.p, c->cy.p, c->cz.p, t);
    launch_nbr_build(st, N, c->cx.p, c->cy.p, c->cz.p, t, c->nbr.p);
    CTX_HIP(c, hipMemsetAsync(c->sh.p, 0, sizeof(float) * 9 * (size_t)N, st));
    size_t sb = 0;
    CTX_HIP(c, rocprim::exclusive_scan(nullptr, sb, c->aflag.p, c->ascan.p, 0, (size_t)N, rocprim::plus<int>(), st));
    c->scan_tmp.release(); CTX_HIP(c, c->scan_tmp.alloc(sb ? sb : 1)); c->scan_tmp_bytes = sb;
    CTX_HIP(c, hipStreamSynchronize(st));
    CTX_HIP(c, hipGetLastError());
    c->have_grid = true;
    return I3D_OK;
}
}

extern "C" {

int i3d_get_grid(i3d_context* c, double* sdf_refined, double* albedo) {
    if (!c || !c->have_grid) return ctx_fail(c, I3D_ERR_STATE, "i3d_get_grid: no grid");
    CTX_HIP(c, hipSetDevice(c->device));
    const int N = c->N;
    DevBuf<double> a, b; CTX_HIP(c, a.alloc(N)); CTX_HIP(c, b.alloc(N));
    launch_gather_visit(c->stream, N, c->rank.p, c->x_sdf.p, c->x_alb.p, a.p, b.p);
    if (sdf_refined) CTX_HIP(c, hipMemcpyAsync(sdf_refined, a.p, sizeof(double) * (size_t)N, hipMemcpyDeviceToHost, c->stream));
    if (albedo) CTX_HIP(c, hipMemcpyAsync(albedo, b.p, sizeof(double) * (size_t)N, hipMemcpyDeviceToHost, c->stream));
    CTX_HIP(c, hipStreamSynchronize(c->stream));
    return I3D_OK;
}

int i3d_update_grid(i3d_context* c, const double* sdf_refined, const double* albedo, const uint8_t* color) {
    if (!c || !c->have_grid) return ctx_fail(c, I3D_ERR_STATE, "i3d_update_grid: no grid");
    CTX_HIP(c, hipSetDevice(c->device));
    const int N = c->N;
    DevBuf<double> a, b; DevBuf<uint8_t> col;
    if (sdf_refined) { CTX_HIP(c, a.alloc(N)); CTX_HIP(c, hipMemcpyAsync(a.p, sdf_refined, sizeof(double) * (size_t)N, hipMemcpyHostToDevice, c->stream)); }
    if (albedo) { CTX_HIP(c, b.alloc(N)); CTX_HIP(c, hipMemcpyAsync(b.p, albedo, sizeof(double) * (size_t)N, hipMemcpyHostToDevice, c->stream)); }
    if (color) { CTX_HIP(c, col.alloc((size_t)3 * N)); CTX_HIP(c, hipMemcpyAsync(col.p, color, (size_t)3 * N, hipMemcpyHostToDevice, c->stream)); }
    launch_update_fields(c->stream, N, c->rank.p, a.p, b.p, col.p, c->x_sdf.p, c->x_alb.p, c->f_sdf.p, c->f_alb.p, c->color.p);
    CTX_HIP(c, hipStreamSynchronize(c->stream));
    c->assembled = false;
    return I3D_OK;
}

int i3d_set_frames(i3d_context* c, int32_t K, int32_t levels, const int32_t* widths, const int32_t* heights,
                   const float* const* lum, const float* const* depth, const uint8_t* const* bgr) {
    if (!c || K <= 0 || levels <= 0 || !widths || !heights || !lum || !depth) return ctx_fail(c, I3D_ERR_INVALID_ARGUMENT, "i3d_set_frames: bad arguments");
    CTX_HIP(c, hipSetDevice(c->device));
    c->have_frames = false; c->K = K; c->levels = levels; c->cull_level = -1;
    c->slots = 0; c->assembled = false;
    c->fw.assign(widths, widths + levels); c->fh.assign(heights, heights + levels);
    c->lum.clear(); c->depth.clear(); c->bgr.clear();
    c->lum.resize((size_t)K * levels); c->depth.resize((size_t)K * levels); c->bgr.resize((size_t)K * levels);
    for (int f = 0; f < K; ++f) for (int l = 0; l < levels; ++l) {
        const size_t k = (size_t)f * levels + l, px = (size_t)widths[l] * heights[l];
        if (!lum[k] || !depth[k]) return ctx_fail(c, I3D_ERR_INVALID_ARGUMENT, "i3d_set_frames: null image");
        CTX_HIP(c, c->lum[k].alloc(px + 4));        CTX_HIP(c, c->depth[k].alloc(px));
        CTX_HIP(c, hipMemcpyAsync(c->lum[k].p, lum[k], px * sizeof(float), hipMemcpyHostToDevice, c->stream));
        CTX_HIP(c, hipMemcpyAsync(c->depth[k].p, depth[k], px * sizeof(float), hipMemcpyHostToDevice, c->stream));
        if (bgr && bgr[k]) { CTX_HIP(c, c->bgr[k].alloc(px * 3)); CTX_HIP(c, hipMemcpyAsync(c->bgr[k].p, bgr[k], px * 3, hipMemcpyHostToDevice, c->stream)); }
    }
    CTX_HIP(c, c->d_frames.alloc(K)); CTX_HIP(c, c->d_frames_cand.alloc(K));
    CTX_HIP(c, hipStreamSynchronize(c->stream));
    c->have_frames = true;
    if ((int)c->poses.size() != 6 * K) { c->poses.assign((size_t)6 * K, 0.0); c->have_camera = false; }
    return I3D_OK;
}

int i3d_set_camera(i3d_context* c, const double* intr, const double* dist, const double* poses) {
    if (!c || !intr || !dist || !poses) return ctx_fail(c, I3D_ERR_INVALID_ARGUMENT, "i3d_set_camera: null pointer");
    if (!c->have_frames) return ctx_fail(c, I3D_ERR_STATE, "i3d_set_camera: set the keyframes first");
    std::memcpy(c->intr, intr, sizeof(double) * 4); std::memcpy(c->dist, dist, sizeof(double) * 5);
    c->poses.assign(poses, poses + (size_t)6 * c->K);
    c->have_camera = true;
    return I3D_OK;
}
int i3d_get_camera(i3d_context* c, double* intr, double* dist, double* poses) {
    if (!c || !c->have_camera) return ctx_fail(c, I3D_ERR_STATE, "i3d_get_camera: no camera");
    if (intr) std::memcpy(intr, c->intr, sizeof(double) * 4);
    if (dist) std::memcpy(dist, c->dist, sizeof(double) * 5);
    if (poses) std::memcpy(poses, c->poses.data(), sizeof(double) * 6 * (size_t)c->K);
    return I3D_OK;
}

int i3d_set_voxel_sh(i3d_context* c, const double* voxel_sh) {
    if (!c || !voxel_sh) return ctx_fail(c, I3D_ERR_INVALID_ARGUMENT, "i3d_set_voxel_sh: null pointer");
    if (!c->have_grid) return ctx_fail(c, I3D_ERR_STATE, "i3d_set_voxel_sh: no grid");
    CTX_HIP(c, hipSetDevice(c->device));
    DevBuf<double> tmp; CTX_HIP(c, tmp.alloc((size_t)9 * c->N));
    CTX_HIP(c, hipMemcpyAsync(tmp.p, voxel_sh, sizeof(double) * 9 * (size_t)c->N, hipMemcpyHostToDevice, c->stream));
    launch_scatter_sh(c->stream, c->N, c->rank.p, tmp.p, c->sh.p);
    CTX_HIP(c, hipStreamSynchronize(c->stream));
// ... 59 lines not shown
```

### intrinsic3d_amd/csrc/host/context.hpp

```cpp
#pragma once
#include <functional>
#include <string>
#include <vector>
#include <cstring>
#include <cmath>
#include "../device/kernels.hpp"
#include "../device/render_kernels.hpp"
#include "../device/track_kernels.hpp"
#include "../device/query_kernels.hpp"
#include "../device/register_kernels.hpp"
#include "../device/track_sdf_kernels.hpp"
#include "comm.hpp"
#include "../../../include/intrinsic3d_hip.h"

namespace i3d {

template <class T>
struct DevBuf {
    T* p = nullptr; size_t n = 0;
    DevBuf() = default;
    DevBuf(const DevBuf&) = delete; DevBuf& operator=(const DevBuf&) = delete;
    DevBuf(DevBuf&& o) noexcept : p(o.p), n(o.n) { o.p = nullptr; o.n = 0; }
    DevBuf& operator=(DevBuf&& o) noexcept { if (this != &o) { release(); p = o.p; n = o.n; o.p = nullptr; o.n = 0; } return *this; }
    ~DevBuf() { release(); }
// ... 60 lines not shown
Pose pose_from_vec6(const double* p6);
void vec6_from_pose(const Pose& P, double* p6);

struct RegisterModel {
    std::function<int(int code, const std::string& msg)> fail;
    std::function<int()> ready;
    std::function<void(const RegisterParams& p, const double* points, const TrackState* state, int check_done, double* slab)> launch;
    double voxel_size;
    int row_cap = REGISTER_MAX_ROWS;
};
int register_run(hipStream_t st, DevBuf<unsigned char>& scratch, const RegisterModel& m, const char* what, const i3d_register_desc* d, int64_t n, const double* points,
                 double* pose6_io, i3d_register_stats* stats, const double* debug_pivot3 = nullptr, double* debug_sums29 = nullptr, int64_t* debug_valid = nullptr);

void pivot_of(const double* sums, const double* R0, const double* t0, double* c);
void start_state(TrackState& hs, const double* R0, const double* t0, const double* c);

struct TrackSdfModel {
    std::function<int(int code, const std::string& msg)> fail;
    std::function<int(const i3d_track_sdf_desc& d, const double*& intr, const double*& dist)> ready;
    std::function<int()> intensity_ready;
    std::function<int(const double*& vol)> intensity;
    std::function<void(const TrackSdfParams& p, const TrackSdfPhoto* ph, const TrackSdfBatch& b, int check_done)> launch;
    double voxel_size;
    int row_cap = REGISTER_MAX_ROWS;
};
struct TrackSdfBuffers { DevBuf<unsigned char> scratch; PinnedBuf staging; };
struct TrackSdfRgbd {
    double geometric_weight, photo_weight; float max_photo_residual;
    i3d_track_sdf_rgbd_stats* stats = nullptr;
};
struct TrackSdfFrames {
    int32_t num, w, h;
    const float* host_depth; const float* const* dev_depth;
    const float* host_lum; const float* const* dev_lum;
};
struct TrackSdfDebug { const double* pivot3; double* sums; int64_t* valid; int64_t* usable; int64_t* photo_samples; };
int track_sdf_chunks(hipStream_t st, TrackSdfBuffers& buf, const TrackSdfModel& m, const i3d_track_sdf_desc* d, const double* intr, const double* dist,
                     const TrackSdfFrames& fr, double* poses6_io, i3d_track_sdf_stats* stats, const TrackSdfRgbd* rgbd = nullptr, int max_chunk = 0,
                     const TrackSdfDebug* debug = nullptr);
int track_sdf_run(hipStream_t st, TrackSdfBuffers& buf, const TrackSdfModel& m, const char* what, const i3d_track_sdf_desc* d, int32_t w, int32_t h,
                  const float* depth, double* pose6_io, i3d_track_sdf_stats* stats, const TrackSdfRgbd* rgbd = nullptr, const float* luminance = nullptr,
                  const TrackSdfDebug* debug = nullptr);

struct SolverSwitches {
    int  deterministic = -1;
    int  ladder = LADDER_MAX;
    bool ladder_mr = true, ladder_mr1 = false, ladder_pair = true; int ladder_group = 3;
    bool egt_mr1 = false;
    int  egt_tile = 0;
    int  hmax_limit = 0, hmax_limit_1024 = 0;
    bool halo_pull = false, no_tile = false, gradcol = true, cost0 = true;
    int  no_cull = 0;
    int  debug_invalid_attempt = -1;
    int  sh_slab = 0;
};

struct Timing {
    bool on = false;
    unsigned mask = ~0u;
    double ms[I3D_K_COUNT] = {0};
    long long launches[I3D_K_COUNT] = {0};
    std::vector<float> each[I3D_K_COUNT];
    struct Pending { hipEvent_t a, b; int cat; };
    std::vector<Pending> pending;
    std::vector<hipEvent_t> pool;
};

}

struct i3d_context {
    int device = 0;
    hipStream_t stream = nullptr;
    std::string err;

    int N = 0; float voxel_size = 0, truncation = 0;
    i3d::DevBuf<int> cx, cy, cz, rank, nbr, aidx, alist, aflag, ascan;
    i3d::DevBuf<double> sdf0, x_sdf, x_alb, xc_sdf, xc_alb;
    i3d::DevBuf<float> f_sdf, f_alb, weight, sh;
    i3d::DevBuf<uchar4> color;
    i3d::DevBuf<uint8_t> flags;
    i3d::DevBuf<unsigned char> scan_tmp; size_t scan_tmp_bytes = 0;
    i3d::DevBuf<unsigned long long> hkeys; i3d::DevBuf<int> hvals; unsigned int hmask = 0;
    bool have_grid = false, have_sh = false;
    i3d::DevBuf<unsigned> render_bits; i3d::DevBuf<int> render_bounds; int render_lo[3] = {0, 0, 0}, render_dim[3] = {0, 0, 0}; bool render_bricks_ok = false;
    i3d::DevBuf<float> render_planes; i3d::DevBuf<i3d::RenderStatsDev> render_stats;
    i3d::TrackBuffers track;
    i3d::DevBuf<unsigned char> query_scratch;
    i3d::DevBuf<unsigned char> register_scratch; int register_row_cap = i3d::REGISTER_MAX_ROWS;
    i3d::TrackSdfBuffers track_sdf; int track_batch_frames = 0;
    i3d::DevBuf<double> track_sdf_intensity;
    std::vector<unsigned long long> sv_keys; std::vector<double> sv_sh; float sv_size = 0.0f; bool have_subvolumes = false;

    int K = 0, levels = 0;
    std::vector<int> fw, fh;
    std::vector<i3d::DevBuf<float>> lum, depth;
    std::vector<i3d::DevBuf<uint8_t>> bgr;
    i3d::DevBuf<i3d::FrameConst> d_frames, d_frames_cand;
    bool have_frames = false;

    double intr[4] = {0, 0, 0, 0}, dist[5] = {0, 0, 0, 0, 0};
    std::vector<double> poses;
    bool have_camera = false;

    int Acap = 0, slots = 0, A = 0; long long n_active = 0;
    i3d::Comm* comm = nullptr; int chunk = 1, own0 = 0, own1 = 0, nC = 0;
    i3d::DevBuf<int> clist, cflag, cscan;
    i3d::HaloPlan halo; i3d::DevBuf<unsigned long long> need_mask, halo_items, halo_sorted; i3d::DevBuf<int> halo_count, halo_send_idx, halo_recv_idx, halo_send_peer, halo_recv_peer, halo_offs, tile_flag, ghost_tiles;
    i3d::DevBuf<float> halo_send_buf, halo_recv_buf; i3d::DevBuf<unsigned char> halo_temp; int n_ghost_tiles = 0, slice = 0;
    i3d::DevBuf<int> obs_frame, anbr; i3d::DevBuf<float> obs_w, ea_w, C, treg;
    i3d::DevBuf<float4> rows; i3d::DevBuf<float2> row_wr;
    i3d::DevBuf<uint8_t> aflags, nrows, regflags, ea_free; i3d::DevBuf<int> gmax;
    i3d::DevBuf<float2> cull_blocks; i3d::DevBuf<float4> cull_bounds; i3d::DevBuf<unsigned> cull_mask; int cull_level = -1; bool cull_on = false;
    double cost_at_build = 0.0;
    i3d::DevBuf<float> C2, treg2, gc_part;
    i3d::DevBuf<float> aux_part;
    i3d::DevBuf<unsigned> tp_lnbr; i3d::DevBuf<int> tp_halo_idx, tp_halo_cnt, tp_iota, tp_ext_e, tp_ext_pos, tp_ext_off, tp_overflow; i3d::DevBuf<float> tp_qh, tp_eaw, cam_part;
    i3d::DevBuf<unsigned char> tp_temp; bool tile_ok = false;
    i3d::DevBuf<unsigned short> tp_hp_off, tp_hp_src; bool halo_pull = false;
    bool ladder_lists = false;
    i3d::SolverSwitches sw;
    bool mr1_serial = false;
    int ladder_max = 1;
    int ladder_hint = 0, ladder_hint_prev = 0;
    i3d::LadVec lad{};
    i3d::DevBuf<float> lad_vec;
    i3d::DevBuf<float> lad_qh, lad_cam, lad_mblk, lad_tail;
    i3d::DevBuf<double> lad_part;
    i3d::DevBuf<double> lad_red;
    i3d::DevBuf<i3d::PcgState> lad_st;
    long long lad_batches = 0, lad_streams = 0, lad_system_passes = 0, lad_resyncs = 0, lad_wasted = 0;
    long long lad_pass_live[7] = {0, 0, 0, 0, 0, 0, 0}, lad_paired = 0;
    double t_add_end = 0.0;
    bool deterministic = false;
    int tile_T = 0;
    int plan_T() const { return tile_T > 0 ? tile_T : (sw.egt_tile == 512 ? 512 : 1024); }
    int plan_hmax_limit() const { return plan_T() == 512 ? sw.hmax_limit : sw.hmax_limit_1024; }
    i3d::TilePlan tile_plan() const {
        const int T = plan_T();
        const bool sh = comm && (comm->world > 1 || comm->force);
        const int t0 = sh ? own0 / T : 0, t1 = sh ? (own1 + T - 1) / T : i3d::tile_plan_tiles_of(A, T);
        return i3d::TilePlan{tp_lnbr.p, tp_eaw.p, tp_halo_idx.p, tp_halo_cnt.p, tp_iota.p, tp_ext_e.p, tp_ext_pos.p, tp_qh.p, tp_ext_off.p, tp_overflow.p, T, i3d::tile_plan_hmax_of(T), t0, t1 > t0 ? t1 - t0 : 0,
                             ghost_tiles.p, sh ? n_ghost_tiles : 0, deterministic ? 1 : 0, (halo_pull || ladder_lists) ? tp_hp_off.p : nullptr, (halo_pull || ladder_lists) ? tp_hp_src.p : nullptr, halo_pull ? 1 : 0};
    }

    i3d::DevBuf<float> v_mask, v_c, v_S, v_cm, v_D2, v_Minv, v_b, v_x, v_r, v_p, v_z, v_q, v_u, v_acc, v_tmp, v_qacc;
    i3d::DevBuf<float> Minv_blocks;
    i3d::DevBuf<double> d_shared, d_blocks, d_scal, d_xshared, d_xcshared;
    i3d::DevBuf<i3d::PcgState> d_pcg, d_pcg2; i3d::DevBuf<double> d_partials; i3d::PcgState* h_pcg = nullptr; hipEvent_t pcg_ev[2] = {nullptr, nullptr};
    int* h_flags = nullptr; int* d_flags = nullptr; int pcg_seq = 1024;
    i3d::DevBuf<i3d::LmState> d_lm; i3d::LmRecord* h_lmrec = nullptr; i3d::LmRecord* d_lmrec = nullptr; int lm_seq = 1;
    i3d::DevBuf<double> d_cam_c, d_cam_H;
    hipEvent_t ev_asm[2] = {nullptr, nullptr};
    long long n_syncs = 0;
    double* h_pinned = nullptr; size_t h_pinned_n = 0;

    i3d::OptParams last_params; bool assembled = false;
    long long last_sizes[6] = {0, 0, 0, 0, 0, 0};
    i3d::Timing timing;

    i3d::GridView grid_view() const;
    i3d::RowView row_view() const;
};

namespace i3d {

int ctx_fail(i3d_context* c, int code, const std::string& msg);
int ctx_hip(i3d_context* c, hipError_t e, const char* what);
int ctx_launch_check(i3d_context* c);
#define CTX_HIP(c, expr) do { hipError_t _e = (expr); if (_e != hipSuccess) return i3d::ctx_hip((c), _e, #expr); } while (0)
void build_frame_consts(const i3d_context* c, int level, const double* poses, std::vector<FrameConst>& out);
int ensure_pinned(i3d_context* c, size_t n);
bool timing_begin(i3d_context* c, int cat);
void timing_end(i3d_context* c);
void timing_flush(i3d_context* c);
struct TimedScope { i3d_context* c; bool active; TimedScope(i3d_context* c_, int cat) : c(c_), active(timing_begin(c_, cat)) {} ~TimedScope() { if (active) timing_end(c); } };

struct GridStaging { DevBuf<int> kxyz; DevBuf<double> sdf, sdf_ref, alb; DevBuf<float> w; DevBuf<uint8_t> rgb; };
int set_grid_device(i3d_context* c, int N, float voxel_size, float truncation, GridStaging& st);

int render_ensure_bricks(i3d_context* c);
RenderGrid render_grid(const i3d_context* c, bool refined);
inline RenderGrid field_grid(const i3d_context* c, bool refined) {
    return RenderGrid{HashTable{c->hkeys.p, c->hvals.p, c->hmask}, c->nbr.p, c->N, c->weight.p, refined ? c->x_sdf.p : c->sdf0.p, c->x_alb.p, c->sh.p,
// ... 20 lines not shown
```

### intrinsic3d_amd/csrc/host/solver.cpp

```cpp
#include "context.hpp"
#include <rocprim/rocprim.hpp>
#include <chrono>
#include <cstdlib>
#include <limits>
#include <algorithm>

namespace i3d {

#ifdef I3D_MR_PHASES
void mr_phase_report_now();
#endif
#ifdef I3D_MR_BLOCKTIME
void mr_blocktime_report_now();
#endif

static double now_s() { return std::chrono::duration<double>(std::chrono::steady_clock::now().time_since_epoch()).count(); }

static OptParams make_params(const i3d_context* c, const i3d_optimizer_config& cfg, const double* intr, const double* dist) {
    OptParams p; std::memset(&p, 0, sizeof(p));
    p.thres_shell = cfg.thres_shell; p.lambda_a = cfg.lambda_a; p.K = c->K; p.level = cfg.rgbd_level;
    p.pyr_scale = 1.0 / std::pow(2.0, cfg.rgbd_level);
    p.occlusion = cfg.occlusion_distance;
    p.use_er = (cfg.lambda_r0 > 0.0 && cfg.lambda_r1 > 0.0); p.use_es = (cfg.lambda_s0 > 0.0 && cfg.lambda_s1 > 0.0); p.use_ea = cfg.lambda_a > 0.0;
    for (int i = 0; i < 4; ++i) { p.intr[i] = intr[i]; p.cam_f[i] = (float)(intr[i] * p.pyr_scale); }
// ... 53 lines not shown
        CTX_HIP(c, c->halo_send_idx.alloc(cap)); CTX_HIP(c, c->halo_recv_idx.alloc(cap)); CTX_HIP(c, c->halo_send_peer.alloc(cap)); CTX_HIP(c, c->halo_recv_peer.alloc(cap)); CTX_HIP(c, c->halo_offs.alloc(2 * P2P_MAX_RANKS)); CTX_HIP(c, c->halo_send_buf.alloc((size_t)HALO_MULTI_MAX * (2 * cap))); CTX_HIP(c, c->halo_recv_buf.alloc((size_t)HALO_MULTI_MAX * (2 * cap)));
        CTX_HIP(c, c->halo_temp.alloc(halo_sort_temp_bytes((int)cap)));
        const size_t nt = (size_t)tile_plan_tiles_of((int)Acap, 512) + 1; CTX_HIP(c, c->tile_flag.alloc(nt)); CTX_HIP(c, c->ghost_tiles.alloc(nt));
    }
    CTX_HIP(c, c->d_scal.alloc(32)); CTX_HIP(c, c->d_xshared.alloc((size_t)6 * c->K + 9)); CTX_HIP(c, c->d_xcshared.alloc((size_t)6 * c->K + 9));
    CTX_HIP(c, c->d_pcg.alloc(1)); CTX_HIP(c, c->d_pcg2.alloc(2));
    CTX_HIP(c, c->d_partials.alloc((Acap / 256 + 2048) * 9));
    if (!c->h_pcg) CTX_HIP(c, hipHostMalloc((void**)&c->h_pcg, 2 * sizeof(PcgState), hipHostMallocDefault));
    for (auto& e : c->pcg_ev) if (!e) CTX_HIP(c, hipEventCreateWithFlags(&e, hipEventDisableTiming));
    if (!c->h_flags) { CTX_HIP(c, hipHostMalloc((void**)&c->h_flags, 32 * sizeof(int), hipHostMallocMapped | hipHostMallocCoherent));
                       for (int i = 0; i < 32; ++i) c->h_flags[i] = -1;
                       CTX_HIP(c, hipHostGetDevicePointer((void**)&c->d_flags, c->h_flags, 0)); }
    CTX_HIP(c, c->d_lm.alloc(1)); CTX_HIP(c, c->d_cam_c.alloc((size_t)6 * c->K + 9)); CTX_HIP(c, c->d_cam_H.alloc((size_t)21 * c->K + 25));
    if (!c->h_lmrec) { CTX_HIP(c, hipHostMalloc((void**)&c->h_lmrec, LM_REC_SLOTS * sizeof(LmRecord), hipHostMallocMapped | hipHostMallocCoherent));
                       std::memset(c->h_lmrec, 0, LM_REC_SLOTS * sizeof(LmRecord));
                       CTX_HIP(c, hipHostGetDevicePointer((void**)&c->d_lmrec, c->h_lmrec, 0)); }
    for (auto& e : c->ev_asm) if (!e) CTX_HIP(c, hipEventCreate(&e));
    return ensure_pinned(c, 64 + (size_t)27 * c->K + 64);
}

struct Layout { int A, K, NS, chunk, world, rank, slice; Seg2 own; size_t tail_off, NP; };
static Layout layout_of(const i3d_context* c) {
    Layout L; L.A = c->A; L.K = c->K; L.NS = 6 * c->K + 9; L.chunk = c->chunk; L.world = c->comm ? c->comm->world : 1; L.rank = c->comm ? c->comm->rank : 0;
    L.slice = L.chunk / L.world;
    L.own = Seg2{(size_t)L.rank * L.slice, (size_t)L.chunk + (size_t)L.rank * L.slice, L.slice};
    L.tail_off = 2 * (size_t)L.chunk; L.NP = L.tail_off + L.NS;
    return L;
}
static bool sharded(const i3d_context* c) { return c->comm && (c->comm->world > 1 || c->comm->force); }
static bool one_stream_gradcol(const i3d_context* c) { return !sharded(c) && c->sw.gradcol; }
static bool cost_from_sums(const i3d_context* c) { return c->sw.cost0 && !one_stream_gradcol(c); }

void read_switches(i3d_context* c) {
    auto env = [](const char* name) { return std::getenv(name); };
    auto is = [&](const char* name, char v) { const char* e = env(name); return e && e[0] == v; };
    auto num = [&](const char* name, int unset) { const char* e = env(name); return e ? std::atoi(e) : unset; };
    auto clamp = [](int v, int lo, int hi) { return v < lo ? lo : (v > hi ? hi : v); };
    SolverSwitches w;
    { const char* e = env("I3D_DETERMINISTIC"); w.deterministic = e ? (e[0] == '1' ? 1 : 0) : -1; }
    w.ladder = clamp(num("I3D_LADDER", LADDER_MAX), 1, LADDER_MAX);
    w.ladder_mr = !is("I3D_LADDER_MR", '0');
    w.ladder_mr1 = is("I3D_LADDER_MR1", '1');
    w.ladder_group = clamp(num("I3D_LADDER_GROUP", 3), 1, 3);
    w.ladder_pair = !is("I3D_LADDER_PAIR", '0');
    w.egt_mr1 = is("I3D_EGT_MR1", '1');
    { const char* e = env("I3D_EGT_TILE"); w.egt_tile = e ? (std::atoi(e) == 512 ? 512 : 1024) : 0; }
    w.hmax_limit = num("I3D_EGT_HMAX_LIMIT", 0);
    w.hmax_limit_1024 = num("I3D_EGT_HMAX_LIMIT_1024", 0);
    w.halo_pull = is("I3D_HALO_PULL", '1');
    w.no_tile = is("I3D_NO_TILE", '1');
    { const char* e = env("I3D_NO_CULL"); w.no_cull = (e && e[0] >= '1' && e[0] <= '3') ? e[0] - '0' : 0; }
    w.gradcol = !is("I3D_GRADCOL", '0');
    w.cost0 = !is("I3D_COST0", '0');
    w.debug_invalid_attempt = num("I3D_DEBUG_INVALID_ATTEMPT", -1);
    { const int v = num("I3D_SH_SLAB", 0); w.sh_slab = v > 0 ? v : 0; }
    c->sw = w;
}

static int allreduce(i3d_context* c, double* dev, size_t n) {
    if (!sharded(c)) return I3D_OK;
    TimedScope t(c, I3D_K_COMM);
    return c->comm->allreduce_sum(dev, n, c->stream) ? ctx_fail(c, I3D_ERR_COMM, "all-reduce failed") : I3D_OK;
}
static int allgather(i3d_context* c, float* vec) {
    if (!sharded(c)) return I3D_OK;
    const size_t slice = (size_t)(c->chunk / c->comm->world);
    TimedScope t(c, I3D_K_COMM);
    if (c->comm->allgather(vec, slice, c->stream) || c->comm->allgather(vec + c->chunk, slice, c->stream)) return ctx_fail(c, I3D_ERR_COMM, "all-gather failed");
    return I3D_OK;
}
static int push_halo(i3d_context* c, float* vec) {
    if (!sharded(c)) return I3D_OK;
    TimedScope t(c, I3D_K_COMM);
    return c->comm->push_halo(vec, c->halo, c->stream) ? ctx_fail(c, I3D_ERR_COMM, "halo exchange failed") : I3D_OK;
}

static int shard_plan(i3d_context* c) {
    hipStream_t s = c->stream;
    const int world = c->comm->world, rank = c->comm->rank;
    if (world > 64) return ctx_fail(c, I3D_ERR_CAPACITY, "sharding: more than 64 ranks");
    shard_range(c->A, world, rank, c->chunk, c->own0, c->own1); c->nC = 0; c->slice = c->chunk / world;
    RowView r0 = c->row_view();
    TimedScope t(c, I3D_K_CLASSIFY);
    launch_mark_compute(s, r0, c->cflag.p);
    CTX_HIP(c, rocprim::exclusive_scan(c->scan_tmp.p, c->scan_tmp_bytes, c->cflag.p, c->cscan.p, 0, (size_t)c->A, rocprim::plus<int>(), s));
    launch_compact_list(s, c->A, c->cflag.p, c->cscan.p, c->clist.p);
    const int T = c->plan_T(), ntiles = tile_plan_tiles_of(c->A, T);
    CTX_HIP(c, hipMemsetAsync(c->need_mask.p, 0, sizeof(unsigned long long) * (size_t)c->A, s));
    CTX_HIP(c, hipMemsetAsync(c->halo_count.p, 0, sizeof(int), s));
    CTX_HIP(c, hipMemsetAsync(c->tile_flag.p, 0, sizeof(int) * (size_t)(ntiles + 1), s));
    launch_need_mask(s, r0, c->slice, c->need_mask.p);
    launch_halo_items(s, c->A, c->slice, rank, c->need_mask.p, c->halo_items.p, c->halo_count.p, HALO_CAP);
    launch_tile_flags(s, c->A, T, c->cflag.p, c->tile_flag.p);
    int tl[2] = {0, 0}, nitems = 0;
    if (c->A > 0) { CTX_HIP(c, hipMemcpyAsync(&tl[0], c->cscan.p + (c->A - 1), sizeof(int), hipMemcpyDeviceToHost, s));
                    CTX_HIP(c, hipMemcpyAsync(&tl[1], c->cflag.p + (c->A - 1), sizeof(int), hipMemcpyDeviceToHost, s)); }
    CTX_HIP(c, hipMemcpyAsync(&nitems, c->halo_count.p, sizeof(int), hipMemcpyDeviceToHost, s));
    std::vector<int> tf((size_t)ntiles + 1, 0);
    CTX_HIP(c, hipMemcpyAsync(tf.data(), c->tile_flag.p, sizeof(int) * (size_t)ntiles, hipMemcpyDeviceToHost, s));
    CTX_HIP(c, sync_stream(c));
    c->nC = tl[0] + tl[1];
    if (nitems > HALO_CAP) return ctx_fail(c, I3D_ERR_CAPACITY, "sharding: the halo plan does not fit its buffers");
    std::vector<int> ghosts; const int t0 = c->own0 / T, t1 = (c->own1 + T - 1) / T;
    for (int i = 0; i < ntiles; ++i) if (tf[i] && (i < t0 || i >= t1)) ghosts.push_back(i);
    c->n_ghost_tiles = (int)ghosts.size();
    if (!ghosts.empty()) CTX_HIP(c, hipMemcpyAsync(c->ghost_tiles.p, ghosts.data(), sizeof(int) * ghosts.size(), hipMemcpyHostToDevice, s));
// ... 353 lines not shown
        const HaloPlan& h = c->halo;
        sa.rim = RimLists{h.n_send, h.n_recv, c->halo_send_idx.p, c->halo_send_peer.p, c->halo_recv_idx.p, c->halo_recv_peer.p, c->halo_offs.p, c->halo_offs.p + P2P_MAX_RANKS};
        sa.n_rim_wg = (h.n_send + h.n_recv) > 0 ? std::max(1, std::min(4, (std::max(h.n_send, h.n_recv) + 1023) / 1024)) : 1;
        sa.zb = c->v_z.p; sa.pb = c->v_p.p; sa.ub = c->v_u.p; sa.cmb = c->v_cm.p; sa.chunk = c->chunk;
    }
    const int wg_cap = sh ? sa.pd.wg_cap : 0;
    PcgState* const st2 = c->d_pcg2.p;
    const int NSP = (L.NS + 3) & ~3;
    double* const step_part = c->d_partials.p; double* const pq_part = c->d_partials.p + 4 * 2048; double* const d2_part = pq_part + 2048;
    { TimedScope t(c, I3D_K_VECTOR); launch_fill(s, (int)L.NP, c->v_x.p, 0.0f); launch_pcg_init3(s, st2, cfg.pcg_fixed_iterations, 500, c->d_lm.p); }
    CTX_HIP(c, hipMemcpyAsync(c->v_r.p, c->v_b.p, sizeof(float) * L.NP, hipMemcpyDeviceToDevice, s));
    Step3Args a = step3_args(c, L, p, tp, c->v_x.p, c->v_r.p, c->v_p.p, c->v_z.p, c->v_qacc.p, tp.qh, step_part, pq_part, d2_part, c->cam_part.p, c->Minv_blocks.p, c->v_D2.p + to, wg_cap);
    a.sharded = sh ? 1 : 0; a.lad_sys = -1;
    int n_step = 0;
    { TimedScope t(c, I3D_K_VECTOR); a.cur = st2; n_step = launch_pcg_step3(s, 0 , a); }
    const bool mr1 = c->mr1_serial && !sh && tp.T == 512 && tp.hp_off != nullptr && r.slots == 5;
    auto op = [&](double* pq, const PcgState* cur) -> int {
        if (mr1) { const int sys0[3] = {0, 0, 0}; LadVec z; std::memset(&z, 0, sizeof(z));
                   return launch_eg_tile_mr(s, r, p, tp, 1, sys0, c->v_u.p, c->v_qacc.p, tp.qh, pq, c->cam_part.p, NSP, cur, z); }
        return launch_eg_tile(s, r, p, c->v_u.p, tp, nullptr, c->v_qacc.p, pq, cur, c->cam_part.p, NSP);
    };
    const int seq0 = c->pcg_seq;
    int it = 1;
    for (;; ++it) {
        PcgState* const prev = st2 + ((it + 1) & 1); PcgState* const cur = st2 + (it & 1);
        sa.seq = seq0 + it; sa.n_slice_partials = a.n_slice_wg; a.sh = sa;
        { TimedScope t(c, I3D_K_VECTOR);
          a.n_d2 = launch_pcg_dir3(s, it == 1, own, to, L.NS, c->v_z.p, c->v_p.p, c->v_S.p, c->v_u.p, c->v_D2.p, c->v_cm.p, c->d_lm.p, step_part, n_step, d2_part, prev, cur, c->d_flags, seq0 + it,
                                   sh ? &sa : nullptr); }
        if (sh) { c->comm->count_reduce(4); c->comm->count_halo(c->halo.n_send); c->comm->count_reduce((size_t)L.NS + 1); }
        { TimedScope t(c, I3D_K_EG_PASS); a.n_pq = op(pq_part, cur); a.n_cam = a.n_pq; }
        a.cur = cur;
        if (it % 10 != 0) { TimedScope t(c, I3D_K_VECTOR); n_step = launch_pcg_step3(s, 1, a); }
        else {
            { TimedScope t(c, I3D_K_VECTOR); launch_pcg_step3(s, 2, a);
              launch_mul2(s, own, c->v_S.p, c->v_x.p, c->v_u.p); launch_mul(s, L.NS, c->v_S.p + to, c->v_x.p + to, c->v_u.p + to); }
            if (sh) { TimedScope t(c, I3D_K_COMM); launch_rim_u(s, sa, cur); c->comm->count_halo(c->halo.n_send); }
            { TimedScope t(c, I3D_K_EG_PASS); a.n_cam = op(nullptr, cur); }
            { TimedScope t(c, I3D_K_VECTOR); n_step = launch_pcg_step3(s, 3, a); }
        }
        if (it >= 2) {
            const int want = seq0 + it - 1; bool done = false;
            { const int rc = wait_pass(c, c->h_flags + 2 * (want & 1), want, "pcg_solve: the device stopped publishing its state", &done); if (rc) return rc; }
            if (done) break;
        }
        if (it > 520) break;
    }
    c->pcg_seq = seq0 + PCG_SEQ_STRIDE;
    *final_state = st2 + (it & 1);
    { const int lrc = ctx_launch_check(c); if (lrc) return lrc; }
    return I3D_OK;
}

constexpr int LAD_PART_STEP = 4 * 2048, LAD_PART_PQ = 2048, LAD_PART_D2 = 2048;
static size_t lad_redop_stride(int NS) { return ((size_t)NS + 1 + 3) & ~(size_t)3; }
static int alloc_ladder(i3d_context* c) {
    const Layout L = layout_of(c);
    const int nsys = c->ladder_max;
    LadVec& lv = c->lad;
    const size_t vec = ((size_t)L.NP + 65535) & ~(size_t)65535;
    const size_t qh = 2 * (size_t)tile_plan_tiles_of((int)std::min((size_t)c->Acap, ((size_t)c->chunk + 65535) & ~(size_t)65535), 512) * (size_t)tile_plan_hmax_of(512);
    const size_t cam = (size_t)2048 * (((size_t)L.NS + 3) & ~(size_t)3);
    lv.vec = vec; lv.qh = qh; lv.cam = cam; lv.part = LAD_PART_STEP + LAD_PART_PQ + LAD_PART_D2; lv.mblk = ((size_t)36 * c->K + 41 + 3) & ~(size_t)3; lv.tail = ((size_t)L.NS + 3) & ~(size_t)3;
    const bool fresh = c->lad_vec.n < (size_t)6 * nsys * vec || !c->lad_vec.p;
    bool ok = c->lad_vec.alloc((size_t)6 * nsys * vec) == hipSuccess;
    if (ok && fresh) ok = hipMemsetAsync(c->lad_vec.p, 0, sizeof(float) * c->lad_vec.n, c->stream) == hipSuccess;
    ok = ok && c->lad_qh.alloc((size_t)nsys * qh) == hipSuccess && c->lad_cam.alloc((size_t)nsys * cam) == hipSuccess && c->lad_part.alloc((size_t)nsys * lv.part) == hipSuccess
            && c->lad_mblk.alloc((size_t)nsys * lv.mblk) == hipSuccess && c->lad_tail.alloc((size_t)nsys * lv.tail) == hipSuccess && c->lad_st.alloc((size_t)2 * LADDER_MAX) == hipSuccess;
    if (ok && sharded(c)) {
        const size_t n = (size_t)LADDER_MAX * (4 + lad_redop_stride(L.NS));
        const bool fresh_r = c->lad_red.n < n || !c->lad_red.p;
        ok = c->lad_red.alloc(n) == hipSuccess;
        if (ok && fresh_r) ok = hipMemsetAsync(c->lad_red.p, 0, sizeof(double) * c->lad_red.n, c->stream) == hipSuccess;
    }
    if (!ok) {
        (void)hipGetLastError();
        c->lad_vec.release(); c->lad_qh.release(); c->lad_cam.release(); c->lad_part.release();
        std::fprintf(stderr, "[i3d] the slabs of the damping ladder (%d systems x %.1f MB) do not fit the device: this outer iteration runs the serial trust-region loop\n", nsys,
                     (double)(6 * vec + qh + cam) * 4.0 / 1e6);
        return 1;
    }
    return I3D_OK;
}
enum { LV_X = 0, LV_R, LV_P, LV_Z, LV_U, LV_Q };
static float* lad_vecp(const i3d_context* c, int kind, int sys = 0) { return c->lad_vec.p + ((size_t)kind * c->ladder_max + sys) * c->lad.vec; }

static int pcg_solve_ladder(i3d_context* c, const i3d_optimizer_config& cfg, const OptParams& p, int B, const PcgState** finals, int* passes_out) {
    hipStream_t s = c->stream;
    const Layout L = layout_of(c);
    const int K = c->K; const size_t to = L.tail_off; const Seg2 own = L.own;
    RowView r = c->row_view(); TilePlan tp = c->tile_plan();
    LadVec lv = c->lad;
    float* const X0 = lad_vecp(c, LV_X); float* const R0 = lad_vecp(c, LV_R); float* const P0 = lad_vecp(c, LV_P); float* const Z0 = lad_vecp(c, LV_Z);
    float* const U0 = lad_vecp(c, LV_U); float* const Q0 = lad_vecp(c, LV_Q);
    PcgState* const st2 = c->lad_st.p;
    const int NSP = (L.NS + 3) & ~3;
    double* const step_part0 = c->lad_part.p; double* const pq_part0 = step_part0 + LAD_PART_STEP; double* const d2_part0 = pq_part0 + LAD_PART_PQ;
    const bool use_mr = c->sw.ladder_mr;
    const bool mr1 = c->sw.ladder_mr1;
    const int mr_cap = std::min(c->sw.ladder_group, eg_tile_mr_max_systems(K));
    const bool pair = c->sw.ladder_pair;
    const bool mr_ok = use_mr && mr_cap >= 1 && tp.T == 512 && tp.hp_off != nullptr && r.slots == 5;
    const bool sh = sharded(c);
    double* const red4 = sh ? c->lad_red.p : nullptr;
    const int rstride = (int)lad_redop_stride(L.NS);
    double* const redop = sh ? c->lad_red.p + (size_t)LADDER_MAX * 4 : nullptr;
    { TimedScope t(c, I3D_K_VECTOR);
      for (int j = 0; j < B; ++j) { CTX_HIP(c, hipMemsetAsync(X0 + (size_t)j * lv.vec, 0, sizeof(float) * L.NP, s));
                                    CTX_HIP(c, hipMemcpyAsync(R0 + (size_t)j * lv.vec, c->v_b.p, sizeof(float) * L.NP, hipMemcpyDeviceToDevice, s)); }
      launch_pcg_init_lad(s, st2, B, cfg.pcg_fixed_iterations, 500, c->d_lm.p); }
    Step3Args a = step3_args(c, L, p, tp, X0, R0, P0, Z0, Q0, c->lad_qh.p, step_part0, pq_part0, d2_part0, c->lad_cam.p, c->lad_mblk.p, c->lad_tail.p, 0);
    a.sharded = 0; a.lad_sys = 0; a.redop = redop; a.redop_stride = rstride;
    std::vector<int> live(B); for (int j = 0; j < B; ++j) live[j] = j;
    auto set_slots = [&]() { for (int q = 0; q < LADDER_MAX; ++q) lv.sysid[q] = live[q < (int)live.size() ? q : (int)live.size() - 1]; };
    auto rows_apply = [&](int parity, bool with_dot) -> int {
        int n = 0; const int nl = (int)live.size();
        if (sh) { TimedScope t(c, I3D_K_COMM);
                  if (c->comm->push_halo_multi(U0, lv.vec, live.data(), nl, c->halo, s)) return -1; }
        if (mr_ok && (nl > 1 || mr1 || sh)) {
            const int groups = (nl + mr_cap - 1) / mr_cap;
            int at = 0;
            if (groups == 2 && pair && !sh && nl - (nl + 1) / 2 >= 2) {
                const int na = (nl + 1) / 2;
                TimedScope t(c, na == 2 ? I3D_K_EG_MR2 : I3D_K_EG_MR3);
                n = launch_eg_tile_mr_pair(s, r, p, tp, na, nl - na, live.data(), U0, Q0, c->lad_qh.p, with_dot ? pq_part0 : nullptr, c->lad_cam.p, NSP, st2 + parity, lv);
                if (n > 0) { at = nl; ++c->lad_streams; ++c->lad_paired; }
// ... 40 lines not shown
          a.n_d2 = launch_pcg_dir3_lad(s, it == 1, nl, own, to, L.NS, Z0, P0, c->v_S.p, U0, c->lad_tail.p, c->v_cm.p, c->d_lm.p, step_part0, n_step, d2_part0, st2, (it + 1) & 1, c->d_flags, seq0 + it, lv,
                                       a.n_slice_wg, red4); }
        { const int n = rows_apply(it & 1, true); if (n < 0) return ctx_fail(c, I3D_ERR_STATE, "pcg_solve_ladder: the multi-system operator pass could not be launched"); a.n_pq = n; a.n_cam = n; }
        a.cur = st2 + (it & 1);
        if (it % 10 != 0) { TimedScope t(c, I3D_K_VECTOR); n_step = launch_pcg_step3_lad(s, 1, nl, a, lv); }
        else {
            { TimedScope t(c, I3D_K_VECTOR); launch_pcg_step3_lad(s, 2, nl, a, lv);
              for (int j : live) { float* xj = X0 + (size_t)j * lv.vec; float* uj = U0 + (size_t)j * lv.vec;
                                   launch_mul2(s, own, c->v_S.p, xj, uj); launch_mul(s, L.NS, c->v_S.p + to, xj + to, uj + to); } }
            { const int n = rows_apply(it & 1, false); if (n < 0) return ctx_fail(c, I3D_ERR_STATE, "pcg_solve_ladder: the multi-system operator pass could not be launched"); a.n_cam = n; }
            { TimedScope t(c, I3D_K_VECTOR); n_step = launch_pcg_step3_lad(s, 3, nl, a, lv); }
        }
        {
            const int want = seq0 + it;
            std::vector<int> still;
            for (int j : live) {
                bool done = false;
                { const int rc = wait_pass(c, c->h_flags + 4 * j + 2 * (want & 1), want, "pcg_solve_ladder: the device stopped publishing its state", &done); if (rc) return rc; }
                if (!done) still.push_back(j);
                else finals[j] = st2 + 2 * j + (it & 1);
            }
            live.swap(still);
            if (live.empty()) break;
        }
        if (it > 520) break;
    }
    if (passes_out) *passes_out = it;
    c->pcg_seq = seq0 + PCG_SEQ_STRIDE;
    for (int j : live) finals[j] = st2 + 2 * j + (it & 1);
    { const int lrc = ctx_launch_check(c); if (lrc) return lrc; }
    return I3D_OK;
}

static int wait_record(i3d_context* c, int idx, int seq, LmRecord& out) {
    LmRecord* const r = c->h_lmrec + idx;
    const double t0 = now_s();
    while (__atomic_load_n(&r->seq, __ATOMIC_ACQUIRE) != seq) {
        if (now_s() - t0 > 60.0) {
            CTX_HIP(c, sync_stream(c));
            if (__atomic_load_n(&r->seq, __ATOMIC_ACQUIRE) != seq) return ctx_fail(c, I3D_ERR_HIP, "lm_solve: the device stopped publishing the state of the trust-region loop");
        }
    }
    out = *r;
    return I3D_OK;
}

static int lm_solve(i3d_context* c, const i3d_optimizer_config& cfg, OptParams& p, i3d_iteration_stats* st, double initial_radius) {
    hipStream_t s = c->stream;
    const Layout L = layout_of(c);
    const int N = c->N, K = c->K, NP = (int)L.NP, NS = L.NS;
    GridView g = c->grid_view(); RowView r = c->row_view();
    if (cfg.lm_steps > LM_REC_SLOTS - 2) return ctx_fail(c, I3D_ERR_CAPACITY, "optimize: more than 62 LM steps per outer iteration");
    { TimedScope t(c, I3D_K_VECTOR); launch_freemask(s, r, p, c->v_mask.p); }
    CTX_HIP(c, hipMemcpyAsync(c->xc_sdf.p, c->x_sdf.p, sizeof(double) * (size_t)N, hipMemcpyDeviceToDevice, s));
    CTX_HIP(c, hipMemcpyAsync(c->xc_alb.p, c->x_alb.p, sizeof(double) * (size_t)N, hipMemcpyDeviceToDevice, s));
    const bool one_stream = one_stream_gradcol(c);
    auto after_colnorm = [&]() -> int {
        CTX_HIP(c, hipMemcpyAsync(c->d_cam_c.p, c->d_shared.p, sizeof(double) * (size_t)NS, hipMemcpyDeviceToDevice, s));
        CTX_HIP(c, hipMemcpyAsync(c->d_cam_H.p, c->d_blocks.p, sizeof(double) * ((size_t)21 * K + 25), hipMemcpyDeviceToDevice, s));
        { int rc2 = allgather(c, c->v_c.p); if (rc2) return rc2; }
        { TimedScope t(c, I3D_K_VECTOR); launch_scale_from_colnorm(s, NP, c->v_c.p, c->v_mask.p, c->v_S.p, c->v_cm.p); }
        return I3D_OK;
    };
    int rc = I3D_OK;
    if (one_stream) { rc = run_gradcol(c, p, after_colnorm); if (rc) return rc; }
    else {
        rc = run_pass(c, PASS_COLNORM, p, nullptr, c->v_c.p); if (rc) return rc;
        rc = after_colnorm(); if (rc) return rc;
        rc = run_pass(c, PASS_GRAD, p, nullptr, c->v_acc.p); if (rc) return rc;
    }
    { TimedScope t(c, I3D_K_VECTOR); launch_mul(s, NP, c->v_S.p, c->v_acc.p, c->v_b.p); }
    if (!c->sw.cost0) { rc = eval_cost_launch(c, p, false, c->d_frames.p); if (rc) return rc; }
    else if (!one_stream) { TimedScope t(c, I3D_K_VECTOR); launch_set_double(s, c->d_scal.p + 16, c->cost_at_build); }
    rc = count_above_dev(c, c->v_acc.p, c->v_mask.p, 1e-10f, c->d_scal.p + 8); if (rc) return rc;
    rc = dot_dev(c, c->v_mask.p, c->v_mask.p, c->d_scal.p + 9); if (rc) return rc;
    {
        double* xs = c->h_pinned;
        for (int i = 0; i < 6 * K; ++i) xs[i] = c->poses[i];
        for (int i = 0; i < 4; ++i) xs[6 * K + i] = c->intr[i];
        for (int i = 0; i < 5; ++i) xs[6 * K + 4 + i] = c->dist[i];
        CTX_HIP(c, hipMemcpyAsync(c->d_xshared.p, xs, sizeof(double) * NS, hipMemcpyHostToDevice, s));
    }
    const int seq0 = c->lm_seq; c->lm_seq += LM_REC_SLOTS;
    LmState* const lm = c->d_lm.p;
    launch_lm_init(s, lm, c->d_scal.p + 16, c->d_scal.p + 8, c->d_scal.p + 9, initial_radius, c->d_lmrec, seq0);

    bool fused = c->tile_ok;
    if (fused && sharded(c)) { P2PDev probe; fused = c->comm->fused_exchange(&probe) && L.NS + 2 <= probe.L.red_cap; }
    int attempts = 0; bool ended = false, accepted = false;
    auto consume = [&](const LmRecord& rec) {
        if (rec.kind == 0) {
            if (st) { st->cost_initial = rec.cost; st->cost_final = rec.cost; st->free_parameters = (int64_t)(rec.nfree + 0.5); st->termination = rec.final_ ? 1 : 0; st->final_radius = initial_radius; }
            c->last_sizes[5] = (long long)(rec.nfree + 0.5);
        } else if (rec.kind == 2) { if (st) st->termination = 1; }
        else {
            if (st) {
                st->lm_iterations = attempts + 1;
                if (attempts < 50) { st->pcg_iterations[attempts] = rec.pcg_it; st->step_accepted[attempts] = rec.accepted; }
                st->final_radius = rec.radius_after; st->termination = rec.termination;
                if (rec.accepted) { st->cost_final = rec.cost; st->successful_steps += 1; }
            }
            if (cfg.verbose) std::printf("  [i3d LM] it %d cand %.9e model %.3e rho %.4f radius -> %.3e cg %d%s\n", attempts + 1, rec.cand_cost, rec.model_change, rec.rel, rec.radius_after, rec.pcg_it,
                                         rec.accepted ? " accepted" : "");
            accepted = rec.accepted != 0;
            ++attempts;
        }
        if (rec.final_) ended = true;
    };
    auto queue_decision = [&](const float* x, const PcgState* ps, int attempt, int lad_next) -> int {
        { TimedScope t(c, I3D_K_VECTOR);
          launch_candidate(s, g, r, K, -1.0f, x, c->v_S.p, c->d_xshared.p, c->xc_sdf.p, c->xc_alb.p, c->d_xcshared.p, c->d_scal.p + 4, c->v_mask.p, c->d_partials.p, lm);
          launch_cand_frames(s, K, c->d_xcshared.p, c->d_frames.p, c->d_frames_cand.p, lm); }
        const int rc2 = eval_cost_launch(c, p, true, c->d_frames_cand.p, c->d_xcshared.p + 6 * K, lm); if (rc2) return rc2;
        { TimedScope t(c, I3D_K_VECTOR);
          launch_lm_decide(s, lm, ps, c->d_scal.p + 4, c->d_scal.p + 16, attempt, cfg.lm_steps, c->d_lmrec + 1 + attempt, seq0 + 1 + attempt, lad_next,
                           c->sw.debug_invalid_attempt == attempt ? 1 : 0);
          launch_accept(s, g, r, c->xc_sdf.p, c->xc_alb.p, lm); }
        return I3D_OK;
    };
    bool ladder = c->ladder_max > 1 && c->tile_ok && (sharded(c) ? !fused : fused) && c->plan_T() == 512 && c->tile_plan().hp_off != nullptr && c->slots == 5;
    if (ladder && alloc_ladder(c) != I3D_OK) {
        ladder = false;
    }
    if (ladder) {
        const LadVec& lv = c->lad;
        { LmRecord rec; rc = wait_record(c, 0, seq0, rec); if (rc) return rc; consume(rec); }
        const bool warm = c->ladder_hint > 0;
        int k = 0, prevB = 0; bool after_resync = false;
        while (k < cfg.lm_steps && !ended) {
            int B = after_resync ? 1 : (prevB == 0 ? (warm ? std::max(c->ladder_hint, c->ladder_hint_prev) : 2) : (warm ? 2 : 2 * prevB));
            B = std::max(1, std::min(B, std::min(c->ladder_max, cfg.lm_steps - k)));
            after_resync = false; prevB = B;
            { TimedScope t(c, I3D_K_VECTOR);
              launch_lm_begin_lad(s, lm, B, K, p.fix_poses, p.fix_intr, p.fix_dist, c->d_cam_c.p, c->d_cam_H.p, c->lad_mblk.p, lv.mblk, c->v_c.p + L.tail_off, c->v_S.p + L.tail_off, c->lad_tail.p, lv.tail,
                                  c->d_lmrec + 1 + k, seq0 + 1 + k); }
            const PcgState* fin[LADDER_MAX] = {nullptr};
            rc = pcg_solve_ladder(c, cfg, p, B, fin, nullptr); if (rc) return rc;
            ++c->lad_batches;
            for (int j = 0; j < B && sharded(c); ++j) { rc = allgather(c, lad_vecp(c, LV_X, j)); if (rc) return rc; }
            for (int j = 0; j < B; ++j) { rc = queue_decision(lad_vecp(c, LV_X, j), fin[j], k + j, j + 1); if (rc) return rc; }
            int decided = 0;
            for (int j = 0; j < B && !ended; ++j) {
                LmRecord rec; rc = wait_record(c, 1 + k + j, seq0 + 1 + k + j, rec); if (rc) return rc;
                if (rec.kind == 3) {
                    __atomic_store_n(&c->h_lmrec[1 + k + j].seq, 0, __ATOMIC_RELEASE);
                    ++c->lad_resyncs; after_resync = true; break;
                }
                consume(rec); ++decided;
            }
            if (ended && decided < B) c->lad_wasted += B - decided;
            k += decided;
        }
        if (attempts > 0) { c->ladder_hint_prev = c->ladder_hint; c->ladder_hint = attempts; }
        ended = true;
    }
    int k = 0;
    for (; !ladder && k < cfg.lm_steps; ++k) {
        { TimedScope t(c, I3D_K_VECTOR);
          launch_lm_begin(s, lm, K, p.fix_poses, p.fix_intr, p.fix_dist, c->d_cam_c.p, c->d_cam_H.p, c->Minv_blocks.p, c->v_c.p + L.tail_off, c->v_S.p + L.tail_off, c->v_D2.p + L.tail_off, c->v_Minv.p + L.tail_off,
                          c->d_lmrec + 1 + k, seq0 + 1 + k);
          if (!fused) launch_lm_diag_dev(s, (int)L.tail_off, c->v_c.p, c->v_S.p, lm, c->v_D2.p, c->v_Minv.p); }
        const PcgState* ps = nullptr;
        rc = fused ? pcg_solve_fused(c, cfg, p, &ps) : pcg_solve(c, cfg, p, &ps); if (rc) return rc;
        { LmRecord rec; rc = wait_record(c, k, seq0 + k, rec); if (rc) return rc; consume(rec); }
        if (ended) break;
        { int rc2 = allgather(c, c->v_x.p); if (rc2) return rc2; }
        rc = queue_decision(c->v_x.p, ps, k, -1); if (rc) return rc;
    }
    if (!ended) { LmRecord rec; rc = wait_record(c, k, seq0 + k, rec); if (rc) return rc; consume(rec); }
    if (st) st->num_attempts = std::min(attempts, 50);
    CTX_HIP(c, hipMemcpyAsync(c->h_pinned, c->d_xcshared.p, sizeof(double) * NS, hipMemcpyDeviceToHost, s));
    CTX_HIP(c, sync_stream(c));
    if (sharded(c) && c->comm->health(s)) return ctx_fail(c, I3D_ERR_COMM, "lm_solve: a peer-to-peer exchange timed out (a rank stopped taking part)");
    if (accepted) {
        for (int i = 0; i < 6 * K; ++i) c->poses[i] = c->h_pinned[i];
        for (int i = 0; i < 4; ++i) c->intr[i] = c->h_pinned[6 * K + i];
        for (int i = 0; i < 5; ++i) c->dist[i] = c->h_pinned[6 * K + 4 + i];
    }
    { const int lrc = ctx_launch_check(c); if (lrc) return lrc; }
    return I3D_OK;
}

int optimize(i3d_context* c, const i3d_optimizer_config& cfg, i3d_iteration_stats* stats) {
    if (!c->have_grid || cfg.iterations < 1) return ctx_fail(c, I3D_ERR_INVALID_ARGUMENT, "optimize: no grid or iterations < 1");
    CTX_HIP(c, hipSetDevice(c->device));
    double carried_radius = 1e4;
    for (int itr = 0; itr < cfg.iterations; ++itr) {
        i3d_iteration_stats local; std::memset(&local, 0, sizeof(local));
        i3d_iteration_stats* st = stats ? &stats[itr] : &local;
        std::memset(st, 0, sizeof(*st));
        OptParams p;
        const double t0 = now_s();
        int rc = assemble(c, cfg, itr, p, st); if (rc) return rc;
        const double t1 = now_s();
        st->time_add = (c->t_add_end >= 0.0 && c->t_add_end <= t1 - t0) ? c->t_add_end : t1 - t0; st->time_build = (t1 - t0) - st->time_add;
        if (c->n_active > 0) { rc = lm_solve(c, cfg, p, st, cfg.carry_trust_radius ? carried_radius : 1e4); if (rc) return rc;
                               if (st->final_radius > 0.0) carried_radius = st->final_radius; }
        const double t2 = now_s();
        st->time_solve = t2 - t1;
        if (cfg.verbose) std::printf("[i3d] itr %d rows %lld/%lld/%lld/%lld valid %lld cost %.9e -> %.9e (add %.3f ms, solve %.3f ms)\n", itr,
                                     (long long)st->rows[0], (long long)st->rows[1], (long long)st->rows[2], (long long)st->rows[3], (long long)st->valid_voxels,
                                     st->cost_initial, st->cost_final, st->time_add * 1e3, st->time_solve * 1e3);
        timing_flush(c);
    }
    c->assembled = false;
#ifdef I3D_MR_PHASES
    mr_phase_report_now();
// ... 69 lines not shown
```

Baseline: 44.09.

## Batch ladder candidate cost evaluation across all LM systems in single launches

```diff
diff --git a/include/intrinsic3d_hip.h b/include/intrinsic3d_hip.h
--- a/include/intrinsic3d_hip.h
+++ b/include/intrinsic3d_hip.h
@@ -408,7 +408,7 @@
 int i3d_debug_jtj_apply(i3d_context* ctx, const double* x, double* y);
 int i3d_debug_work_list(i3d_context* ctx, int32_t* visit_index , int64_t capacity, int64_t* count);
 int i3d_debug_counters(i3d_context* ctx, int64_t* stream_syncs);
-int i3d_debug_ladder_stats(i3d_context* ctx, int64_t* out6);
+int i3d_debug_ladder_stats(i3d_context* ctx, int64_t* out8);
 int i3d_debug_ladder_passes(i3d_context* ctx, int64_t* out8);
 #define I3D_LM_SCRIPT_GUARD 64
 typedef struct i3d_lm_script_desc {
diff --git a/intrinsic3d_amd/binding.py b/intrinsic3d_amd/binding.py
--- a/intrinsic3d_amd/binding.py
+++ b/intrinsic3d_amd/binding.py
@@ -954,9 +954,10 @@
         return {"stream_syncs": int(n.value)}
 
     def debug_ladder_stats(self):
-        a = (C.c_int64 * 6)()
+        a = (C.c_int64 * 8)()
         self._check(self.L.i3d_debug_ladder_stats(self.h, a), "i3d_debug_ladder_stats")
-        return {"batches": int(a[0]), "row_streams": int(a[1]), "system_passes": int(a[2]), "resyncs": int(a[3]), "unused_systems": int(a[4]), "depth": int(a[5])}
+        return {"batches": int(a[0]), "row_streams": int(a[1]), "system_passes": int(a[2]), "resyncs": int(a[3]), "unused_systems": int(a[4]), "depth": int(a[5]),
+                "cost_launches": int(a[6]), "cost_candidates": int(a[7])}
 
     def debug_ladder_passes(self):
         a = (C.c_int64 * 8)()
diff --git a/intrinsic3d_amd/csrc/device/build.hip b/intrinsic3d_amd/csrc/device/build.hip
--- a/intrinsic3d_amd/csrc/device/build.hip
+++ b/intrinsic3d_amd/csrc/device/build.hip
@@ -167,7 +167,7 @@
     return (one_minus < 0.01f) ? 0.01f : one_minus;
 }
 
-template <bool WITH_J, bool FR_LDS, int BATCH> __global__ void k_build(GridView g, RowView r, OptParams p, const FrameConst* __restrict__ frames, double* cost_out, const double* __restrict__ cam9, const LmState* __restrict__ lm);
+template <bool WITH_J, bool FR_LDS, int BATCH> __global__ void k_build(GridView g, RowView r, OptParams p, const FrameConst* __restrict__ frames, double* cost_out, const double* __restrict__ cam9, const LmState* __restrict__ lm, CandBatch cb);
 #ifdef I3D_BUILD_VALUE_PROBE
 constexpr int BUILD_PROBE_WAVES = I3D_BUILD_VALUE_PROBE;
 #else
@@ -175,10 +175,20 @@
 #endif
 template <bool WITH_J, bool FR_LDS, int BATCH>
 __global__ void __launch_bounds__(256, WITH_J ? (BUILD_PROBE_WAVES ? BUILD_PROBE_WAVES : 2) : 3) k_build(GridView g, RowView r, OptParams p, const FrameConst* __restrict__ frames, double* cost_out,
-                                                               const double* __restrict__ cam9, const LmState* __restrict__ lm) {
+                                                               const double* __restrict__ cam9, const LmState* __restrict__ lm, CandBatch cb) {
     extern __shared__ double frame_lds_raw[];
+    int bx = blockIdx.x;
     if (!WITH_J) {
         if (lm && lm->done) return;
+        if (cb.B > 0) {
+            const int grp = (int)blockIdx.x / (8 * cb.B), rr = (int)blockIdx.x % (8 * cb.B), j = rr / 8;
+            bx = grp * 8 + (rr % 8);
+            if (bx * (int)blockDim.x >= r.nC) return;
+            if (lm->lad_radius[j] < 1e-32) return;
+            g.x_sdf = cb.xc_sdf + (size_t)j * cb.xc; g.x_alb = cb.xc_alb + (size_t)j * cb.xc;
+            frames = cb.frames + (size_t)j * cb.fr; cam9 = cb.xsh + (size_t)j * cb.sh + 6 * p.K;
+            cost_out = cb.part + (size_t)j * cb.part_stride + CAND_PART_NORMS;
+        }
         if (cam9) { for (int i = 0; i < 4; ++i) p.intr[i] = cam9[i]; for (int i = 0; i < 5; ++i) p.dist[i] = cam9[4 + i]; }
     }
     FrameHot* const flds = reinterpret_cast<FrameHot*>(frame_lds_raw);
@@ -190,17 +200,7 @@
         }
         __syncthreads();
     }
-#ifdef I3D_COST_MULTI_PROBE
-    int bx = blockIdx.x; bool probe_extra = false;
-#ifdef I3D_COST_MULTI_PROBE_FAR
-    if (!WITH_J) { constexpr int PB = I3D_COST_MULTI_PROBE; const int per = (int)gridDim.x / PB; probe_extra = (int)blockIdx.x / per != 0; bx = (int)blockIdx.x % per; }
-#else
-    if (!WITH_J) { constexpr int PB = I3D_COST_MULTI_PROBE; const int grp = (int)blockIdx.x / (8 * PB), rr = (int)blockIdx.x % (8 * PB); probe_extra = rr / 8 != 0; bx = grp * 8 + (rr % 8); }
-#endif
     const int ci = bx * blockDim.x + threadIdx.x;
-#else
-    const int ci = blockIdx.x * blockDim.x + threadIdx.x;
-#endif
     const int a = ci < r.nC ? (r.clist ? r.clist[ci] : ci) : -1;
     const bool owned = a >= r.own0 && a < r.own1;
     double cost = 0.0;
@@ -498,37 +498,39 @@
         }
         }
     }
-#ifdef I3D_COST_MULTI_PROBE
-    if (!WITH_J && probe_extra) cost = 0.0;
-#endif
-    if (!WITH_J) block_partial_d(cost, cost_out, 1, 0);
+    if (!WITH_J) { const double t = block_sum_d(cost); if (threadIdx.x == 0) cost_out[bx] = t; }
 }
 
 void launch_build(hipStream_t st, GridView g, RowView r, OptParams p, const FrameConst* frames, bool with_jacobian, double* cost_out, double* scratch,
                   const double* cam9, const LmState* lm) {
     if (r.nC <= 0) { if (!with_jacobian && cost_out) (void)hipMemsetAsync(cost_out, 0, sizeof(double), st); return; }
-#ifdef I3D_COST_MULTI_PROBE
-    const int blocks = with_jacobian ? (r.nC + 255) / 256 : (((r.nC + 255) / 256 + 7) / 8) * 8 * I3D_COST_MULTI_PROBE;
-#else
     const int blocks = (r.nC + 255) / 256;
-#endif
     double* const cost_dst = cost_out; cost_out = scratch;
     const size_t lds = (size_t)p.K * sizeof(FrameHot), qlds = (size_t)256 * Q_LDS_STRIDE;
     if (with_jacobian) {
 #ifdef I3D_BUILD_VALUE_PROBE
         if (BUILD_PROBE_WAVES > 2) {
             if (!set_dynamic_lds((const void*)k_build<true, true, 2>, "k_build<true> value probe", lds, p.K)) return;
-            k_build<true, true, 2><<<blocks, 256, lds, st>>>(g, r, p, frames, cost_out, nullptr, nullptr);
+            k_build<true, true, 2><<<blocks, 256, lds, st>>>(g, r, p, frames, cost_out, nullptr, nullptr, CandBatch{});
             return;
         }
 #endif
         if (!set_dynamic_lds((const void*)k_build<true, false, 2>, "k_build<true>", qlds, p.K)) return;
-        k_build<true, false, 2><<<blocks, 256, qlds, st>>>(g, r, p, frames, cost_out, nullptr, nullptr);
+        k_build<true, false, 2><<<blocks, 256, qlds, st>>>(g, r, p, frames, cost_out, nullptr, nullptr, CandBatch{});
     } else {
-        if (lds <= 48 * 1024) k_build<false, true, 2><<<blocks, 256, lds, st>>>(g, r, p, frames, cost_out, cam9, lm);
-        else k_build<false, false, 2><<<blocks, 256, 0, st>>>(g, r, p, frames, cost_out, cam9, lm);
+        if (lds <= 48 * 1024) k_build<false, true, 2><<<blocks, 256, lds, st>>>(g, r, p, frames, cost_out, cam9, lm, CandBatch{});
+        else k_build<false, false, 2><<<blocks, 256, 0, st>>>(g, r, p, frames, cost_out, cam9, lm, CandBatch{});
     }
     if (!with_jacobian) launch_reduce_partials(st, scratch, blocks, 1, cost_dst, nullptr, true);
+}
+
+int launch_build_cost_lad(hipStream_t st, GridView g, RowView r, OptParams p, CandBatch cb, const LmState* lm) {
+    if (r.nC <= 0 || cb.B <= 0) return 0;
+    const int vb = (r.nC + 255) / 256, blocks = ((vb + 7) / 8) * 8 * cb.B;
+    const size_t lds = (size_t)p.K * sizeof(FrameHot);
+    if (lds <= 48 * 1024) k_build<false, true, 2><<<blocks, 256, lds, st>>>(g, r, p, nullptr, nullptr, nullptr, lm, cb);
+    else k_build<false, false, 2><<<blocks, 256, 0, st>>>(g, r, p, nullptr, nullptr, nullptr, lm, cb);
+    return vb;
 }
 
 template <bool COST>
diff --git a/intrinsic3d_amd/csrc/device/common.hpp b/intrinsic3d_amd/csrc/device/common.hpp
--- a/intrinsic3d_amd/csrc/device/common.hpp
+++ b/intrinsic3d_amd/csrc/device/common.hpp
@@ -138,7 +138,8 @@
     int invalid;
     int attempts;
     int successful;
-    double lad_radius[LADDER_MAX]; float lad_inv_radius[LADDER_MAX]; int lad_n; int pad1;
+    double lad_radius[LADDER_MAX]; float lad_inv_radius[LADDER_MAX]; int lad_n;
+    int lad_accept;
 };
 struct LmRecord {
     int seq; int final_;
diff --git a/intrinsic3d_amd/csrc/device/kernels.hpp b/intrinsic3d_amd/csrc/device/kernels.hpp
--- a/intrinsic3d_amd/csrc/device/kernels.hpp
+++ b/intrinsic3d_amd/csrc/device/kernels.hpp
@@ -31,6 +31,16 @@
 
 void launch_build(hipStream_t st, GridView g, RowView r, OptParams p, const FrameConst* frames, bool with_jacobian, double* cost_out , double* scratch,
                   const double* cam9 = nullptr, const LmState* lm = nullptr);
+constexpr int CAND_PART_NORMS = 2 * 1024;
+struct CandBatch {
+    int B;
+    double* xc_sdf; double* xc_alb; size_t xc;
+    double* xsh; size_t sh;
+    FrameConst* frames; size_t fr;
+    double* part; size_t part_stride;
+    double* scal;
+};
+int  launch_build_cost_lad(hipStream_t st, GridView g, RowView r, OptParams p, CandBatch cb, const LmState* lm);
 void launch_weight_sums(hipStream_t st, RowView r, GridView g, bool with_cost, double* sums13 , double* scratch);
 
 enum PassMode { PASS_GRAD = 0, PASS_JTJP = 1, PASS_COLNORM = 2 };
@@ -176,6 +186,11 @@
 void launch_candidate(hipStream_t st, GridView g, RowView r, int K, float sign, const float* step, const float* S, const double* x_shared, double* xc_sdf, double* xc_alb,
                       double* xc_shared, double* norms2 , const float* mask, double* scratch, const LmState* lm = nullptr);
 void launch_accept(hipStream_t st, GridView g, RowView r, const double* xc_sdf, const double* xc_alb, const LmState* lm = nullptr);
+int  launch_candidate_lad(hipStream_t st, GridView g, RowView r, int K, float sign, const float* step0, size_t step_stride, const float* S, const double* x_shared, const float* mask,
+                          CandBatch cb, const LmState* lm);
+void launch_reduce_cand(hipStream_t st, CandBatch cb, int n_norm, int n_cost, const LmState* lm);
+void launch_accept_lad(hipStream_t st, GridView g, RowView r, int K, CandBatch cb, double* xc_shared_out, const LmState* lm);
+void launch_cand_mirror_fix(hipStream_t st, GridView g, int A_prev, const int* alist_prev, const int* aidx, CandBatch cb, int nsys);
 void launch_set_double(hipStream_t st, double* dst, double v);
 void launch_lm_init(hipStream_t st, LmState* lm, const double* cost, const double* ngrad, const double* nfree, double radius0, LmRecord* rec, int seq);
 void launch_lm_begin(hipStream_t st, LmState* lm, int K, int fix_poses, int fix_intr, int fix_dist, const double* cdiag, const double* tri, float* Mblk,
@@ -184,6 +199,10 @@
 void launch_cand_frames(hipStream_t st, int K, const double* xc, const FrameConst* base, FrameConst* out, const LmState* lm);
 void launch_lm_decide(hipStream_t st, LmState* lm, const PcgState* ps, const double* norms2, const double* cand_cost, int attempt, int lm_steps, LmRecord* rec, int seq,
                       int lad_next = -1 , int debug_invalid = 0);
+struct PcgFinals { const PcgState* p[LADDER_MAX]; };
+void launch_cand_frames_lad(hipStream_t st, int K, const FrameConst* base, CandBatch cb, const LmState* lm);
+void launch_lm_decide_lad(hipStream_t st, LmState* lm, PcgFinals fin, const double* scal , int B, int attempt0, int lm_steps, LmRecord* rec, int seq,
+                          int debug_invalid_attempt);
 void launch_lm_begin_lad(hipStream_t st, LmState* lm, int B, int K, int fix_poses, int fix_intr, int fix_dist, const double* cdiag, const double* tri, float* Mblk, size_t mblk_stride,
                          const float* tc, const float* tS, float* tD2, size_t tail_stride, LmRecord* rec, int seq);
 void launch_mark_compute(hipStream_t st, RowView r, int* flag);
diff --git a/intrinsic3d_amd/csrc/device/lm_kernels.hip b/intrinsic3d_amd/csrc/device/lm_kernels.hip
--- a/intrinsic3d_amd/csrc/device/lm_kernels.hip
+++ b/intrinsic3d_amd/csrc/device/lm_kernels.hip
@@ -135,9 +135,8 @@
     if (K > 0) k_cand_frames<<<(K + 63) / 64, 64, 0, st>>>(K, xc, base, out, lm);
 }
 
-__global__ void k_lm_decide(LmState* lm, const PcgState* __restrict__ ps, const double* __restrict__ norms2, const double* __restrict__ cand_cost_p, int attempt , int lm_steps,
-                            LmRecord* rec, int seq, int lad_next, int debug_invalid) {
-    if (lm->done) return;
+static __device__ inline void lm_decide_one(LmState* lm, const PcgState* ps, const double* norms2, const double* cand_cost_p, int attempt , int lm_steps,
+                                            LmRecord* rec, int seq, int lad_next, int debug_invalid) {
     const int pcg_it = ps->done == 2 ? ps->it + 1 : ps->it;
     const double xbr = ps->xbr, d2xx = ps->d2xx;
     const double model_change = 0.5 * xbr + 0.5 * d2xx;
@@ -186,8 +185,38 @@
         }
     }
 }
+__global__ void k_lm_decide(LmState* lm, const PcgState* ps, const double* norms2, const double* cand_cost_p, int attempt, int lm_steps, LmRecord* rec, int seq, int lad_next, int debug_invalid) {
+    if (lm->done) return;
+    lm_decide_one(lm, ps, norms2, cand_cost_p, attempt, lm_steps, rec, seq, lad_next, debug_invalid);
+}
 void launch_lm_decide(hipStream_t st, LmState* lm, const PcgState* ps, const double* norms2, const double* cand_cost, int attempt, int lm_steps, LmRecord* rec, int seq, int lad_next, int debug_invalid) {
     k_lm_decide<<<1, 1, 0, st>>>(lm, ps, norms2, cand_cost, attempt, lm_steps, rec, seq, lad_next, debug_invalid);
 }
 
-}
+__global__ void __launch_bounds__(64) k_cand_frames_lad(int K, const FrameConst* __restrict__ base, CandBatch cb, const LmState* __restrict__ lm) {
+    const int j = blockIdx.y;
+    if (lm->done || lm->lad_radius[j] < 1e-32) return;
+    const int f = blockIdx.x * blockDim.x + threadIdx.x;
+    if (f >= K) return;
+    FrameConst fc = base[f];
+    double p[6];
+    for (int i = 0; i < 6; ++i) p[i] = cb.xsh[(size_t)j * cb.sh + 6 * f + i];
+    fm::frame_from_pose(p, fc);
+    cb.frames[(size_t)j * cb.fr + f] = fc;
+}
+void launch_cand_frames_lad(hipStream_t st, int K, const FrameConst* base, CandBatch cb, const LmState* lm) {
+    if (K > 0 && cb.B > 0) k_cand_frames_lad<<<dim3((K + 63) / 64, cb.B), 64, 0, st>>>(K, base, cb, lm);
+}
+__global__ void k_lm_decide_lad(LmState* lm, PcgFinals fin, const double* scal, int B, int attempt0, int lm_steps, LmRecord* rec, int seq, int debug_invalid_attempt) {
+    lm->lad_accept = -1;
+    for (int j = 0; j < B; ++j) {
+        if (lm->done) return;
+        lm_decide_one(lm, fin.p[j], scal + 4 * j, scal + 4 * j + 2, attempt0 + j, lm_steps, rec + j, seq + j, j + 1, debug_invalid_attempt == attempt0 + j ? 1 : 0);
+        if (lm->accepted) lm->lad_accept = j;
+    }
+}
+void launch_lm_decide_lad(hipStream_t st, LmState* lm, PcgFinals fin, const double* scal, int B, int attempt0, int lm_steps, LmRecord* rec, int seq, int debug_invalid_attempt) {
+    k_lm_decide_lad<<<1, 1, 0, st>>>(lm, fin, scal, B, attempt0, lm_steps, rec, seq, debug_invalid_attempt);
+}
+
+}
diff --git a/intrinsic3d_amd/csrc/device/operator.hip b/intrinsic3d_amd/csrc/device/operator.hip
--- a/intrinsic3d_amd/csrc/device/operator.hip
+++ b/intrinsic3d_amd/csrc/device/operator.hip
@@ -7,8 +7,7 @@
 #define GRID_STRIDE(n) const int stride = gridDim.x * blockDim.x; for (int i = blockIdx.x * blockDim.x + threadIdx.x; i < (n); i += stride)
 static inline int vblocks(int n) { int b = (n + 255) / 256; return b < 1 ? 1 : (b > 2048 ? 2048 : b); }
 
-__global__ void __launch_bounds__(1024) k_reduce_partials(const double* __restrict__ partials, int nblk, int ncomp, double* dst, const PcgState* __restrict__ state, int assign) {
-    if (state && state->done) return;
+static __device__ inline void reduce_partials_wg(const double* __restrict__ partials, int nblk, int ncomp, double* dst, int assign) {
     for (int k = 0; k < ncomp; ++k) {
         double s = 0.0;
         for (int i0 = threadIdx.x; i0 < nblk; i0 += 8 * 1024) {
@@ -21,6 +20,20 @@
         const double t = block_sum_d(s);
         if (threadIdx.x == 0) dst[k] = assign ? t : dst[k] + t;
     }
+}
+__global__ void __launch_bounds__(1024) k_reduce_partials(const double* __restrict__ partials, int nblk, int ncomp, double* dst, const PcgState* __restrict__ state, int assign) {
+    if (state && state->done) return;
+    reduce_partials_wg(partials, nblk, ncomp, dst, assign);
+}
+__global__ void __launch_bounds__(1024) k_reduce_cand(CandBatch cb, int n_norm, int n_cost, const LmState* __restrict__ lm) {
+    const int j = blockIdx.x;
+    if (lm->done || lm->lad_radius[j] < 1e-32) return;
+    const double* const part = cb.part + (size_t)j * cb.part_stride;
+    if (blockIdx.y == 0) reduce_partials_wg(part, n_norm, 2, cb.scal + 4 * j, 1);
+    else reduce_partials_wg(part + CAND_PART_NORMS, n_cost, 1, cb.scal + 4 * j + 2, 1);
+}
+void launch_reduce_cand(hipStream_t st, CandBatch cb, int n_norm, int n_cost, const LmState* lm) {
+    if (cb.B > 0) k_reduce_cand<<<dim3(cb.B, 2), 1024, 0, st>>>(cb, n_norm, n_cost, lm);
 }
 void launch_reduce_partials(hipStream_t st, const double* partials, int nblk, int ncomp, double* dst, const PcgState* state, bool assign) {
     if (nblk > 0) k_reduce_partials<<<1, 1024, 0, st>>>(partials, nblk, ncomp, dst, state, assign ? 1 : 0);
@@ -834,6 +847,79 @@
 }
 void launch_accept(hipStream_t st, GridView g, RowView r, const double* xc_sdf, const double* xc_alb, const LmState* lm) { if (r.A > 0) k_accept<<<vblocks(r.A), 256, 0, st>>>(g, r, xc_sdf, xc_alb, lm); }
 
+__global__ void __launch_bounds__(256) k_candidate_lad(GridView g, RowView r, int K, float sign, const float* __restrict__ step0, size_t step_stride, const float* __restrict__ S,
+                                                       const double* __restrict__ xsh, const float* __restrict__ mask, CandBatch cb, const LmState* __restrict__ lm) {
+    if (lm->done) return;
+    const int A = r.A, NS = 6 * K + 9, chunk = r.chunk;
+    const size_t tail = 2 * (size_t)chunk;
+    bool live[LADDER_MAX]; double d2[LADDER_MAX];
+#pragma unroll
+    for (int j = 0; j < LADDER_MAX; ++j) { live[j] = j < cb.B && !(lm->lad_radius[j] < 1e-32); d2[j] = 0.0; }
+    double x2 = 0.0;
+    GRID_STRIDE(A + NS) {
+        if (i < A) {
+            const int s = r.alist[i]; const int js = vec_sdf(i, chunk), ja = js + chunk;
+            const double Ss = (double)S[js], Sa = (double)S[ja];
+            const double xs = g.x_sdf[s], xa = g.x_alb[s];
+            const bool ms = mask[js] != 0.0f, ma = mask[ja] != 0.0f;
+#pragma unroll
+            for (int j = 0; j < LADDER_MAX; ++j) if (live[j]) {
+                const float* const step = step0 + (size_t)j * step_stride;
+                const double ds = (double)sign * (double)step[js] * Ss, da = (double)sign * (double)step[ja] * Sa;
+                cb.xc_sdf[(size_t)j * cb.xc + s] = xs + ds; cb.xc_alb[(size_t)j * cb.xc + s] = xa + da;
+                if (ms) d2[j] += ds * ds;
+                if (ma) d2[j] += da * da;
+            }
+            if (ms) x2 += xs * xs;
+            if (ma) x2 += xa * xa;
+        } else {
+            const int t = i - A; const size_t jt = tail + t;
+            const double St = (double)S[jt], x = xsh[t];
+            const bool mt = mask[jt] != 0.0f;
+#pragma unroll
+            for (int j = 0; j < LADDER_MAX; ++j) if (live[j]) {
+                const double delta = (double)sign * (double)step0[(size_t)j * step_stride + jt] * St;
+                cb.xsh[(size_t)j * cb.sh + t] = x + delta;
+                if (mt) d2[j] += delta * delta;
+            }
+            if (mt) x2 += x * x;
+        }
+    }
+#pragma unroll
+    for (int j = 0; j < LADDER_MAX; ++j) if (live[j]) {
+        double* const part = cb.part + (size_t)j * cb.part_stride;
+        block_partial_d(d2[j], part, 2, 0); block_partial_d(x2, part, 2, 1);
+    }
+}
+int launch_candidate_lad(hipStream_t st, GridView g, RowView r, int K, float sign, const float* step0, size_t step_stride, const float* S, const double* xsh, const float* mask,
+                         CandBatch cb, const LmState* lm) {
+    if (cb.B <= 0) return 0;
+    int b = vblocks(r.A + 6 * K + 9); if (b > 1024) b = 1024;
+    k_candidate_lad<<<b, 256, 0, st>>>(g, r, K, sign, step0, step_stride, S, xsh, mask, cb, lm);
+    return b;
+}
+__global__ void k_accept_lad(GridView g, RowView r, int NS, CandBatch cb, double* __restrict__ xc_shared_out, const LmState* __restrict__ lm) {
+    const int acc = lm->lad_accept;
+    if (acc < 0) return;
+    if (blockIdx.x == 0) for (int t = threadIdx.x; t < NS; t += blockDim.x) xc_shared_out[t] = cb.xsh[(size_t)acc * cb.sh + t];
+    const double* const xc_sdf = cb.xc_sdf + (size_t)acc * cb.xc; const double* const xc_alb = cb.xc_alb + (size_t)acc * cb.xc;
+    GRID_STRIDE(r.A) { const int s = r.alist[i]; const double a = xc_sdf[s], b = xc_alb[s]; g.x_sdf[s] = a; g.x_alb[s] = b; g.f_sdf[s] = (float)a; g.f_alb[s] = (float)b; }
+}
+__global__ void k_cand_mirror_fix(GridView g, int A_prev, const int* __restrict__ alist_prev, const int* __restrict__ aidx, CandBatch cb, int nsys) {
+    GRID_STRIDE(A_prev) {
+        const int s = alist_prev[i];
+        if (aidx[s] >= 0) continue;
+        const double a = g.x_sdf[s], b = g.x_alb[s];
+        for (int j = 0; j < nsys; ++j) { cb.xc_sdf[(size_t)j * cb.xc + s] = a; cb.xc_alb[(size_t)j * cb.xc + s] = b; }
+    }
+}
+void launch_cand_mirror_fix(hipStream_t st, GridView g, int A_prev, const int* alist_prev, const int* aidx, CandBatch cb, int nsys) {
+    if (A_prev > 0 && nsys > 0) k_cand_mirror_fix<<<vblocks(A_prev), 256, 0, st>>>(g, A_prev, alist_prev, aidx, cb, nsys);
+}
+void launch_accept_lad(hipStream_t st, GridView g, RowView r, int K, CandBatch cb, double* xc_shared_out, const LmState* lm) {
+    if (cb.B > 0) k_accept_lad<<<vblocks(r.A), 256, 0, st>>>(g, r, 6 * K + 9, cb, xc_shared_out, lm);
+}
+
 __global__ void k_halo_pack(int n, const int* __restrict__ idx, const float* __restrict__ vec, int chunk, float* __restrict__ buf) {
     const int i = blockIdx.x * blockDim.x + threadIdx.x;
     if (i < n) { const int e = idx[i]; buf[2 * (size_t)i] = vec[e]; buf[2 * (size_t)i + 1] = vec[(size_t)chunk + e]; }
diff --git a/intrinsic3d_amd/csrc/host/capi.cpp b/intrinsic3d_amd/csrc/host/capi.cpp
--- a/intrinsic3d_amd/csrc/host/capi.cpp
+++ b/intrinsic3d_amd/csrc/host/capi.cpp
@@ -194,9 +194,10 @@
     return I3D_OK;
 }
 
-int i3d_debug_ladder_stats(i3d_context* c, int64_t* out6) {
-    if (!c || !out6) return I3D_ERR_INVALID_ARGUMENT;
-    out6[0] = c->lad_batches; out6[1] = c->lad_streams; out6[2] = c->lad_system_passes; out6[3] = c->lad_resyncs; out6[4] = c->lad_wasted; out6[5] = c->ladder_max;
+int i3d_debug_ladder_stats(i3d_context* c, int64_t* out8) {
+    if (!c || !out8) return I3D_ERR_INVALID_ARGUMENT;
+    out8[0] = c->lad_batches; out8[1] = c->lad_streams; out8[2] = c->lad_system_passes; out8[3] = c->lad_resyncs; out8[4] = c->lad_wasted; out8[5] = c->ladder_max;
+    out8[6] = c->lad_cost_launches; out8[7] = c->lad_cost_cands;
     return I3D_OK;
 }
 int i3d_debug_ladder_passes(i3d_context* c, int64_t* out8) {
diff --git a/intrinsic3d_amd/csrc/host/context.cpp b/intrinsic3d_amd/csrc/host/context.cpp
--- a/intrinsic3d_amd/csrc/host/context.cpp
+++ b/intrinsic3d_amd/csrc/host/context.cpp
@@ -165,6 +165,7 @@
                         c->x_sdf.p, c->x_alb.p, c->f_sdf.p, c->f_alb.p, c->weight.p, c->color.p);
     CTX_HIP(c, hipMemcpyAsync(c->xc_sdf.p, c->x_sdf.p, sizeof(double) * (size_t)N, hipMemcpyDeviceToDevice, st));
     CTX_HIP(c, hipMemcpyAsync(c->xc_alb.p, c->x_alb.p, sizeof(double) * (size_t)N, hipMemcpyDeviceToDevice, st));
+    c->cand_mirror_N = 0;
     unsigned int cap = 1; while (cap < (unsigned int)N * 2u) cap <<= 1;
     CTX_HIP(c, fit(c->hkeys, cap)); CTX_HIP(c, fit(c->hvals, cap)); c->hmask = cap - 1;
     CTX_HIP(c, hipMemsetAsync(c->hkeys.p, 0xff, sizeof(unsigned long long) * (size_t)cap, st));
@@ -205,6 +206,7 @@
     if (albedo) { CTX_HIP(c, b.alloc(N)); CTX_HIP(c, hipMemcpyAsync(b.p, albedo, sizeof(double) * (size_t)N, hipMemcpyHostToDevice, c->stream)); }
     if (color) { CTX_HIP(c, col.alloc((size_t)3 * N)); CTX_HIP(c, hipMemcpyAsync(col.p, color, (size_t)3 * N, hipMemcpyHostToDevice, c->stream)); }
     launch_update_fields(c->stream, N, c->rank.p, a.p, b.p, col.p, c->x_sdf.p, c->x_alb.p, c->f_sdf.p, c->f_alb.p, c->color.p);
+    c->cand_mirror_N = 0;
     CTX_HIP(c, hipStreamSynchronize(c->stream));
     c->assembled = false;
     return I3D_OK;
diff --git a/intrinsic3d_amd/csrc/host/context.hpp b/intrinsic3d_amd/csrc/host/context.hpp
--- a/intrinsic3d_amd/csrc/host/context.hpp
+++ b/intrinsic3d_amd/csrc/host/context.hpp
@@ -136,6 +136,7 @@
     bool halo_pull = false, no_tile = false, gradcol = true, cost0 = true;
     int  no_cull = 0;
     int  debug_invalid_attempt = -1;
+    bool cost_batch = true;
     int  sh_slab = 0;
 };
 
@@ -212,7 +213,11 @@
     i3d::DevBuf<double> lad_part;
     i3d::DevBuf<double> lad_red;
     i3d::DevBuf<i3d::PcgState> lad_st;
+    i3d::DevBuf<double> lad_xc, lad_xcsh, lad_cpart, lad_cscal; i3d::DevBuf<i3d::FrameConst> lad_frames; size_t lad_cpart_stride = 0;
+    i3d::DevBuf<int> lad_alist_prev; int cand_prev_A = 0;
+    int cand_mirror_N = 0, cand_mirror_B = 0;
     long long lad_batches = 0, lad_streams = 0, lad_system_passes = 0, lad_resyncs = 0, lad_wasted = 0;
+    long long lad_cost_launches = 0, lad_cost_cands = 0;
     long long lad_pass_live[7] = {0, 0, 0, 0, 0, 0, 0}, lad_paired = 0;
     double t_add_end = 0.0;
     bool deterministic = false;
diff --git a/intrinsic3d_amd/csrc/host/solver.cpp b/intrinsic3d_amd/csrc/host/solver.cpp
--- a/intrinsic3d_amd/csrc/host/solver.cpp
+++ b/intrinsic3d_amd/csrc/host/solver.cpp
@@ -129,6 +129,7 @@
     { const char* e = env("I3D_NO_CULL"); w.no_cull = (e && e[0] >= '1' && e[0] <= '3') ? e[0] - '0' : 0; }
     w.gradcol = !is("I3D_GRADCOL", '0');
     w.cost0 = !is("I3D_COST0", '0');
+    w.cost_batch = !is("I3D_COST_BATCH", '0');
     w.debug_invalid_attempt = num("I3D_DEBUG_INVALID_ATTEMPT", -1);
     { const int v = num("I3D_SH_SLAB", 0); w.sh_slab = v > 0 ? v : 0; }
     c->sw = w;
@@ -588,6 +589,7 @@
     return I3D_OK;
 }
 
+static bool cost_batch_on(const i3d_context* c) { return c->sw.cost_batch && !sharded(c); }
 constexpr int LAD_PART_STEP = 4 * 2048, LAD_PART_PQ = 2048, LAD_PART_D2 = 2048;
 static size_t lad_redop_stride(int NS) { return ((size_t)NS + 1 + 3) & ~(size_t)3; }
 static int alloc_ladder(i3d_context* c) {
@@ -608,6 +610,15 @@
         const bool fresh_r = c->lad_red.n < n || !c->lad_red.p;
         ok = c->lad_red.alloc(n) == hipSuccess;
         if (ok && fresh_r) ok = hipMemsetAsync(c->lad_red.p, 0, sizeof(double) * c->lad_red.n, c->stream) == hipSuccess;
+    }
+    if (ok && cost_batch_on(c)) {
+        const size_t N = (size_t)c->N, cpart = (size_t)CAND_PART_NORMS + (size_t)c->Acap / 256 + 2048;
+        if (c->lad_xc.n < 2 * nsys * N || !c->lad_xc.p) c->cand_mirror_N = 0;
+        ok = c->lad_xc.alloc(2 * nsys * N) == hipSuccess && c->lad_xcsh.alloc((size_t)nsys * lv.tail) == hipSuccess && c->lad_frames.alloc((size_t)nsys * c->K) == hipSuccess
+             && c->lad_cpart.alloc((size_t)nsys * std::max(cpart, c->lad_cpart_stride)) == hipSuccess && c->lad_cscal.alloc((size_t)4 * LADDER_MAX) == hipSuccess
+             && c->lad_alist_prev.alloc(N) == hipSuccess;
+        if (ok) c->lad_cpart_stride = std::max(cpart, c->lad_cpart_stride);
+        else { c->lad_xc.release(); c->cand_mirror_N = 0; }
     }
     if (!ok) {
         (void)hipGetLastError();
@@ -754,8 +765,6 @@
     GridView g = c->grid_view(); RowView r = c->row_view();
     if (cfg.lm_steps > LM_REC_SLOTS - 2) return ctx_fail(c, I3D_ERR_CAPACITY, "optimize: more than 62 LM steps per outer iteration");
     { TimedScope t(c, I3D_K_VECTOR); launch_freemask(s, r, p, c->v_mask.p); }
-    CTX_HIP(c, hipMemcpyAsync(c->xc_sdf.p, c->x_sdf.p, sizeof(double) * (size_t)N, hipMemcpyDeviceToDevice, s));
-    CTX_HIP(c, hipMemcpyAsync(c->xc_alb.p, c->x_alb.p, sizeof(double) * (size_t)N, hipMemcpyDeviceToDevice, s));
     const bool one_stream = one_stream_gradcol(c);
     auto after_colnorm = [&]() -> int {
         CTX_HIP(c, hipMemcpyAsync(c->d_cam_c.p, c->d_shared.p, sizeof(double) * (size_t)NS, hipMemcpyDeviceToDevice, s));
@@ -824,6 +833,48 @@
     if (ladder && alloc_ladder(c) != I3D_OK) {
         ladder = false;
     }
+    const bool cost_batch = ladder && cost_batch_on(c);
+    CandBatch cand{};
+    if (!cost_batch) {
+        c->cand_mirror_N = 0;
+        CTX_HIP(c, hipMemcpyAsync(c->xc_sdf.p, c->x_sdf.p, sizeof(double) * (size_t)N, hipMemcpyDeviceToDevice, s));
+        CTX_HIP(c, hipMemcpyAsync(c->xc_alb.p, c->x_alb.p, sizeof(double) * (size_t)N, hipMemcpyDeviceToDevice, s));
+    } else {
+        const int nsys = c->ladder_max;
+        cand.B = 0; cand.xc_sdf = c->lad_xc.p; cand.xc_alb = c->lad_xc.p + (size_t)nsys * N; cand.xc = (size_t)N;
+        cand.xsh = c->lad_xcsh.p; cand.sh = c->lad.tail; cand.frames = c->lad_frames.p; cand.fr = (size_t)K;
+        cand.part = c->lad_cpart.p; cand.part_stride = c->lad_cpart_stride; cand.scal = c->lad_cscal.p;
+        if (c->cand_mirror_N != N || c->cand_mirror_B != nsys) {
+            c->cand_mirror_N = 0;
+            for (int j = 0; j < nsys; ++j) {
+                CTX_HIP(c, hipMemcpyAsync(cand.xc_sdf + (size_t)j * N, c->x_sdf.p, sizeof(double) * (size_t)N, hipMemcpyDeviceToDevice, s));
+                CTX_HIP(c, hipMemcpyAsync(cand.xc_alb + (size_t)j * N, c->x_alb.p, sizeof(double) * (size_t)N, hipMemcpyDeviceToDevice, s));
+            }
+            c->cand_mirror_B = nsys;
+        } else { TimedScope t(c, I3D_K_VECTOR); launch_cand_mirror_fix(s, g, c->cand_prev_A, c->lad_alist_prev.p, c->aidx.p, cand, nsys); }
+        c->cand_mirror_N = 0;
+    }
+    auto mirror_kept = [&]() -> int {
+        if (!cost_batch) return I3D_OK;
+        if (r.A > 0) CTX_HIP(c, hipMemcpyAsync(c->lad_alist_prev.p, r.alist, sizeof(int) * (size_t)r.A, hipMemcpyDeviceToDevice, s));
+        c->cand_prev_A = r.A; c->cand_mirror_N = N;
+        return I3D_OK;
+    };
+    auto queue_batch = [&](int B, const PcgState* const* fin, int k) -> int {
+        CandBatch cb = cand; cb.B = B;
+        PcgFinals pf; for (int j = 0; j < LADDER_MAX; ++j) pf.p[j] = fin[j < B ? j : 0];
+        int n_norm = 0, n_cost = 0;
+        { TimedScope t(c, I3D_K_VECTOR);
+          n_norm = launch_candidate_lad(s, g, r, K, -1.0f, lad_vecp(c, LV_X), c->lad.vec, c->v_S.p, c->d_xshared.p, c->v_mask.p, cb, lm);
+          launch_cand_frames_lad(s, K, c->d_frames.p, cb, lm); }
+        { TimedScope t(c, I3D_K_COST); n_cost = launch_build_cost_lad(s, g, r, p, cb, lm); }
+        { TimedScope t(c, I3D_K_VECTOR);
+          launch_reduce_cand(s, cb, n_norm, n_cost, lm);
+          launch_lm_decide_lad(s, lm, pf, cb.scal, B, k, cfg.lm_steps, c->d_lmrec + 1 + k, seq0 + 1 + k, c->sw.debug_invalid_attempt);
+          launch_accept_lad(s, g, r, K, cb, c->d_xcshared.p, lm); }
+        ++c->lad_cost_launches; c->lad_cost_cands += B;
+        return I3D_OK;
+    };
     if (ladder) {
         const LadVec& lv = c->lad;
         { LmRecord rec; rc = wait_record(c, 0, seq0, rec); if (rc) return rc; consume(rec); }
@@ -840,7 +891,8 @@
             rc = pcg_solve_ladder(c, cfg, p, B, fin, nullptr); if (rc) return rc;
             ++c->lad_batches;
             for (int j = 0; j < B && sharded(c); ++j) { rc = allgather(c, lad_vecp(c, LV_X, j)); if (rc) return rc; }
-            for (int j = 0; j < B; ++j) { rc = queue_decision(lad_vecp(c, LV_X, j), fin[j], k + j, j + 1); if (rc) return rc; }
+            if (cost_batch) { rc = queue_batch(B, fin, k); if (rc) return rc; }
+            for (int j = 0; j < B && !cost_batch; ++j) { rc = queue_decision(lad_vecp(c, LV_X, j), fin[j], k + j, j + 1); if (rc) return rc; }
             int decided = 0;
             for (int j = 0; j < B && !ended; ++j) {
                 LmRecord rec; rc = wait_record(c, 1 + k + j, seq0 + 1 + k + j, rec); if (rc) return rc;
@@ -855,6 +907,7 @@
         }
         if (attempts > 0) { c->ladder_hint_prev = c->ladder_hint; c->ladder_hint = attempts; }
         ended = true;
+        rc = mirror_kept(); if (rc) return rc;
     }
     int k = 0;
     for (; !ladder && k < cfg.lm_steps; ++k) {
```

Measured after the change: 45.02 (median of 6 runs). 1.02x the previous value.
